# ZhengyiLuo/PULSE

Hardware: NVIDIA H100
Metric: env-steps/sec at 16384 humanoid envs, 1/2/4/8 H100; obs-kernel HBM GB/s (higher is better)
Workload: dtype bf16 GEMM operands, fp32 accumulate / master weights / observations

## Files before the change

pulse_b200/csrc/gemm_kernel.inc:

```
#if PULSE_GEMM_GROUPED
#define PULSE_GEMM_FIRST(member) grp.p[0].member
#define PULSE_GEMM_W wl
#define PULSE_GEMM_SELECT(w)                                                                                         \
  int pi = 0;                                                                                                        \
  while (pi + 1 < grp.count && (w) >= grp.p[pi].item_end) ++pi;                                                      \
  const GemmProblem& P = grp.p[pi];                                                                                  \
  const int wl = (w) - (pi == 0 ? 0 : grp.p[pi - 1].item_end);                                                       \
  const CUtensorMap& map_a = P.map_a;                                                                                \
  const CUtensorMap& map_b = P.map_b;                                                                                \
  const CUtensorMap& map_c = P.map_c;                                                                                \
  const CUtensorMap& map_p = P.map_p;                                                                                \
  const int tma_out = P.tma_out;                                                                                     \
  const pulse_gemm_epilogue_t& ep = P.ep;                                                                            \
  const int M = P.M, N = P.N, K = P.K, kb_per_split = P.kb_per_split;                                                \
  const int tiles_n = (N + BN - 1) / BN, tiles_m = (M + BM - 1) / BM;                                                \
  const int tiles = tiles_m * tiles_n;                                                                               \
  const int num_kb_total = (K + BK - 1) / BK;                                                                        \
  (void)map_a; (void)map_b; (void)map_c; (void)map_p; (void)tma_out; (void)ep; (void)M; (void)N; (void)tiles_n; (void)kb_per_split; (void)num_kb_total;
#else
#define PULSE_GEMM_FIRST(member) member
#define PULSE_GEMM_W w
#define PULSE_GEMM_SELECT(w)
#endif

#if PULSE_GEMM_GROUPED
template <bool A_MN, bool B_MN, int MODE>
__global__ void __launch_bounds__(kThreads, 1) gemm_bf16_grouped_kernel(const __grid_constant__ GemmGroup grp) {
#else
template <bool A_MN, bool B_MN, int MODE>
__global__ void __launch_bounds__(kThreads, 1) gemm_bf16_kernel(const __grid_constant__ CUtensorMap map_a,
                                                                const __grid_constant__ CUtensorMap map_b,
                                                                const __grid_constant__ CUtensorMap map_c,
                                                                const __grid_constant__ CUtensorMap map_p,
                                                                const pulse_gemm_epilogue_t ep, int M, int N, int K,
                                                                int kb_per_split, int splits, int tma_out) {
#endif
  constexpr bool kFwd = MODE == kModeGeneric || MODE == kModeFwd;
  constexpr bool kDgrad = MODE == kModeGeneric || MODE == kModeDgrad || MODE == kModeDgradVec;
  constexpr bool kGateVec = MODE == kModeGeneric || MODE == kModeDgradVec;
  constexpr bool kAccum = MODE == kModeGeneric || MODE == kModeWgrad;
  constexpr bool kBf16Out = MODE != kModeWgrad;
  constexpr bool kRegEpi = MODE == kModeFwd || MODE == kModeDgrad;
  extern __shared__ unsigned char gsm_raw[];
  GemmSmem& sm = *reinterpret_cast<GemmSmem*>((reinterpret_cast<uintptr_t>(gsm_raw) + 1023) & ~static_cast<uintptr_t>(1023));
  const int warp = threadIdx.x >> 5, lane = threadIdx.x & 31;
  const int work0 = static_cast<int>(blockIdx.x);
  const int work_stride = static_cast<int>(gridDim.x);
#if PULSE_GEMM_GROUPED
  const int total = grp.total_items;
#else
  const int tiles_n = (N + BN - 1) / BN, tiles_m = (M + BM - 1) / BM;
  const int tiles = tiles_m * tiles_n;
  const int total = tiles * splits;
  const int num_kb_total = (K + BK - 1) / BK;
#endif
  if (threadIdx.x == 0) PULSE_TRACE(0);

  if (threadIdx.x == 0) {
#pragma unroll
    for (int s = 0; s < kStages; ++s) {
      g_mbar_init(&sm.full[s], 1);
      g_mbar_init(&sm.empty[s], kConsumerWarps);
    }
    asm volatile("fence.mbarrier_init.release.cluster;\n" ::: "memory");
    asm volatile("prefetch.tensormap [%0];\n" ::"l"(&PULSE_GEMM_FIRST(map_a)) : "memory");
    asm volatile("prefetch.tensormap [%0];\n" ::"l"(&PULSE_GEMM_FIRST(map_b)) : "memory");
  }
  __syncthreads();
  if (threadIdx.x == 0) PULSE_TRACE(1);
  asm volatile("griddepcontrol.launch_dependents;\n" ::: "memory");

  if (warp < 4) {
    if (warp == 0 && lane == 0) {
      asm volatile("griddepcontrol.wait;\n" ::: "memory");
      PULSE_TRACE(2);
      int it = 0;
      for (int w = work0; w < total; w += work_stride) {
        PULSE_GEMM_SELECT(w)
        const int split = PULSE_GEMM_W / tiles, t = PULSE_GEMM_W - split * tiles;
        const int m0 = (t / tiles_n) * BM, n0 = (t % tiles_n) * BN;
        const int kb0 = split * kb_per_split;
        const int num_kb = min(kb_per_split, num_kb_total - kb0);
        for (int kb = 0; kb < num_kb; ++kb, ++it) {
          const int s = it % kStages;
          g_mbar_wait(&sm.empty[s], ((it / kStages) & 1) ^ 1);
          g_mbar_expect_tx(&sm.full[s], kStageBytesA + kStageBytesB);
          const int kk = (kb0 + kb) * BK;
          if (A_MN) {
            tma_load_2d(sm.a[s], &map_a, m0, kk, &sm.full[s]);
            tma_load_2d(sm.a[s] + 8192, &map_a, m0 + 64, kk, &sm.full[s]);
          } else {
            tma_load_2d(sm.a[s], &map_a, kk, m0, &sm.full[s]);
          }
          if (B_MN) {
            tma_load_2d(sm.b[s], &map_b, n0, kk, &sm.full[s]);
            tma_load_2d(sm.b[s] + 8192, &map_b, n0 + 64, kk, &sm.full[s]);
          } else {
            tma_load_2d(sm.b[s], &map_b, kk, n0, &sm.full[s]);
          }
        }
      }
    }
  } else {
    const int wg = (warp >> 2) - 1;
    const int ew = warp - 4;
    const int quarter = wg * 2 + (warp & 1);
    const int chalf = (warp >> 1) & 1;
    float* red_stage = sm.red[ew];
    float* acc_s = sm.acc[wg];
    asm volatile("griddepcontrol.wait;\n" ::: "memory");
    int it = 0, lw = 0;
    for (int w = work0; w < total; w += work_stride, ++lw) {
      PULSE_GEMM_SELECT(w)
      const int split = PULSE_GEMM_W / tiles, t = PULSE_GEMM_W - split * tiles;
      const int m0 = (t / tiles_n) * BM, n0 = (t % tiles_n) * BN;
      const int kb0 = split * kb_per_split;
      const int num_kb = min(kb_per_split, num_kb_total - kb0);
      const bool reg_epi = kRegEpi && tma_out;
      const int r0 = (warp & 3) * 16 + (lane >> 2);
      const int row = m0 + quarter * 32 + lane;
      const bool row_ok = row < M;
      const bool gate_fast = (MODE == kModeGeneric || MODE == kModeDgrad) && ep.gate != nullptr && ep.gate_mask == nullptr && ep.gate_mode == PULSE_ACT_RELU && (ep.ldg & 7) == 0 && n0 + chalf * kCols + kCols <= N;
      unsigned gmask[8] = {};
      const bool gate_bits = kDgrad && ep.gate_mask != nullptr;
      if (gate_bits && reg_epi) {
#pragma unroll
        for (int c = 0; c < 4; ++c) {
#pragma unroll
          for (int h = 0; h < 2; ++h) {
            const int r = m0 + wg * 64 + r0 + 8 * h;
            if (r < M && n0 + c * 32 < N) gmask[2 * c + h] = __ldg(ep.gate_mask + static_cast<long long>((n0 >> 5) + c) * ep.ld_gmask + r);
          }
        }
      } else if (gate_bits && row_ok) {
#pragma unroll
        for (int cc = 0; cc < kChunks; ++cc) {
          const int col = n0 + (chalf * kChunks + cc) * 32;
          if (col < N) gmask[cc] = __ldg(ep.gate_mask + static_cast<long long>(col >> 5) * ep.ld_gmask + row);
        }
      }
      if (gate_fast && row_ok) {
        const uint4* g = reinterpret_cast<const uint4*>(reinterpret_cast<const __nv_bfloat16*>(ep.gate) + static_cast<long long>(row) * ep.ldg +
                                                        n0 + chalf * kCols);
        uint4 u[kChunks * 4];
#pragma unroll
        for (int i = 0; i < kChunks * 4; ++i) u[i] = __ldg(g + i);
#pragma unroll
        for (int i = 0; i < kChunks * 4; ++i) {
          const unsigned wds[4] = {u[i].x, u[i].y, u[i].z, u[i].w};
#pragma unroll
          for (int q = 0; q < 4; ++q) {
            const unsigned pos = (((wds[q] & 0x7fff7fffu) + 0x7fff7fffu) & ~wds[q]) & 0x80008000u;
            gmask[i >> 2] |= (pos >> 15) << ((i & 3) * 4 + q);
          }
        }
      }
      const bool gate_vec = kGateVec && ep.gate != nullptr && !gate_fast && !gate_bits && (ep.ldg & 7) == 0;
      uint4 gq[4] = {};
      auto gate_fetch = [&](int cc) {
        const int c0 = n0 + cc * 32;
        if (gate_vec && row_ok && c0 + 32 <= N) {
          const uint4* g = reinterpret_cast<const uint4*>(reinterpret_cast<const __nv_bfloat16*>(ep.gate) + static_cast<long long>(row) * ep.ldg + c0);
#pragma unroll
          for (int q = 0; q < 4; ++q) gq[q] = __ldg(g + q);
        }
      };
      gate_fetch(chalf * kChunks);
      float bias_l[kChunks] = {};
      if (reg_epi && kFwd && ep.bias != nullptr) {
        const int t = (warp & 3) * 32 + lane;
        sm.bias[wg][t] = n0 + t < N ? __ldg(ep.bias + n0 + t) : 0.0f;
      } else if (kFwd && ep.bias != nullptr) {
#pragma unroll
        for (int cc = 0; cc < kChunks; ++cc) {
          const int col = n0 + (chalf * kChunks + cc) * 32 + lane;
          if (col < N) bias_l[cc] = __ldg(ep.bias + col);
        }
      }

      float d[64];
#pragma unroll
      for (int i = 0; i < 64; ++i) d[i] = 0.0f;
      acc_fence(d);
      int prev_s = -1;
      for (int kb = 0; kb < num_kb; ++kb, ++it) {
        const int s = it % kStages;
        g_mbar_wait(&sm.full[s], (it / kStages) & 1);
        if (it == 0 && ew == 0 && lane == 0) PULSE_TRACE(3);
        wgmma_fence();
        const unsigned a_addr = s_u32(sm.a[s]) + static_cast<unsigned>(wg) * 8192u, b_addr = s_u32(sm.b[s]);
#pragma unroll
        for (int k = 0; k < BK / MMA_K; ++k) {
          const unsigned long long da = A_MN ? gmma_desc(a_addr + k * 2048, 8192) : gmma_desc(a_addr + k * 32, 16);
          const unsigned long long db = B_MN ? gmma_desc(b_addr + k * 2048, 8192) : gmma_desc(b_addr + k * 32, 16);
          wgmma_m64n128<A_MN ? 1 : 0, B_MN ? 1 : 0>(d, da, db, (kb | k) != 0 ? 1u : 0u);
        }
        wgmma_commit();
        wgmma_wait<1>();
        if (prev_s >= 0 && lane == 0) g_mbar_arrive(&sm.empty[prev_s]);
        prev_s = s;
      }
      wgmma_wait<0>();
      acc_fence(d);
      if (lane == 0) g_mbar_arrive(&sm.empty[prev_s]);
      if (ew == 0 && lane == 0 && lw < 3) PULSE_TRACE(4 + lw);

      if (kRegEpi && (warp & 3) == 0 && lane == 0) asm volatile("cp.async.bulk.wait_group.read 0;\n" ::: "memory");
      wg_sync(wg);
      float sq = 0.0f;

      if (reg_epi) {
        const int q = lane & 3;
        if (ep.alpha != 1.0f) {
#pragma unroll
          for (int i = 0; i < 64; ++i) d[i] *= ep.alpha;
        }
        if (kFwd && ep.bias != nullptr) {
          const float* bs = sm.bias[wg] + 2 * q;
#pragma unroll
          for (int j = 0; j < BN / 8; ++j) {
            const float2 b = *reinterpret_cast<const float2*>(bs + 8 * j);
            d[4 * j] += b.x; d[4 * j + 1] += b.y; d[4 * j + 2] += b.x; d[4 * j + 3] += b.y;
          }
        }
        if (kFwd && ep.relu_mask != nullptr) {
          unsigned wd[4][2];
#pragma unroll
          for (int c = 0; c < 4; ++c) {
#pragma unroll
            for (int h = 0; h < 2; ++h) {
              unsigned b = 0u;
#pragma unroll
              for (int jj = 0; jj < 4; ++jj)
#pragma unroll
                for (int e = 0; e < 2; ++e) b |= (d[4 * (4 * c + jj) + 2 * h + e] > 0.0f ? 1u : 0u) << (8 * jj + e);
              wd[c][h] = b << (2 * q);
            }
          }
          const bool up2 = (q & 2) != 0, up1 = (q & 1) != 0;
          unsigned wf[2];
#pragma unroll
          for (int h = 0; h < 2; ++h) {
            unsigned w2[2];
#pragma unroll
            for (int k = 0; k < 2; ++k) w2[k] = (up2 ? wd[k + 2][h] : wd[k][h]) | __shfl_xor_sync(0xffffffffu, up2 ? wd[k][h] : wd[k + 2][h], 2);
            wf[h] = (up1 ? w2[1] : w2[0]) | __shfl_xor_sync(0xffffffffu, up1 ? w2[0] : w2[1], 1);
          }
          const int col0 = n0 + 32 * q;
          if (col0 < N) {
            const unsigned valid = N - col0 >= 32 ? 0xffffffffu : (1u << (N - col0)) - 1u;
#pragma unroll
            for (int h = 0; h < 2; ++h) {
              const int r = m0 + wg * 64 + r0 + 8 * h;
              if (r < M) ep.relu_mask[static_cast<long long>(col0 >> 5) * ep.ld_rmask + r] = wf[h] & valid;
            }
          }
        }
        if (gate_bits) {
#pragma unroll
          for (int c = 0; c < 4; ++c) {
#pragma unroll
            for (int h = 0; h < 2; ++h) {
              const unsigned mk = gmask[2 * c + h] >> (2 * q);
#pragma unroll
              for (int jj = 0; jj < 4; ++jj)
#pragma unroll
                for (int e = 0; e < 2; ++e) {
                  float& x = d[4 * (4 * c + jj) + 2 * h + e];
                  x = ((mk >> (8 * jj + e)) & 1u) ? x : 0.0f;
                }
            }
          }
        }
        if (kDgrad && ep.sumsq != nullptr) {
#pragma unroll
          for (int i = 0; i < 64; ++i) sq = fmaf(d[i], d[i], sq);
        }
        const unsigned stage = s_u32(acc_s);
        const bool pre = kFwd && ep.preact != nullptr;
        if (!kFwd || ep.act == PULSE_ACT_NONE) stage_tile_bf16<PULSE_ACT_NONE>(d, stage, pre, n0, N);
        else if (ep.act == PULSE_ACT_RELU) stage_tile_bf16<PULSE_ACT_RELU>(d, stage, pre, n0, N);
        else stage_tile_bf16<PULSE_ACT_SILU>(d, stage, pre, n0, N);
        asm volatile("fence.proxy.async.shared::cta;\n" ::: "memory");
        wg_sync(wg);
        if (ew == 0 && lane == 0 && lw < 3) PULSE_TRACE(16 + 2 * lw);
        if ((warp & 3) == 0 && lane == 0 && m0 + wg * 64 < M) {
#pragma unroll
          for (int b = 0; b < 2; ++b) {
            if (n0 + 64 * b >= N) continue;
            tma_store_2d(&map_c, stage + b * 8192, n0 + 64 * b, m0 + wg * 64);
            if (pre) tma_store_2d(&map_p, stage + 16384 + b * 8192, n0 + 64 * b, m0 + wg * 64);
          }
          asm volatile("cp.async.bulk.commit_group;\n" ::: "memory");
        }
        if (kDgrad && ep.sumsq != nullptr) add_sumsq(ep.sumsq, sq);
        if (ew == 0 && lane == 0 && lw < 3) PULSE_TRACE(17 + 2 * lw);
        continue;
      }

      {
#pragma unroll
        for (int j = 0; j < BN / 8; ++j) {
          const int col = 8 * j + 2 * (lane & 3);
#pragma unroll
          for (int h = 0; h < 2; ++h) {
            const int r = r0 + 8 * h;
            const int rb = r & 31;
            float* blk = acc_s + ((r >> 5) * 4 + (col >> 5)) * 1024;
            const int unit = ((col & 31) >> 2) ^ (rb & 7);
            *reinterpret_cast<float2*>(blk + rb * 32 + unit * 4 + (col & 3)) = make_float2(d[4 * j + 2 * h], d[4 * j + 2 * h + 1]);
          }
        }
      }
      if (MODE == kModeWgrad && tma_out) asm volatile("fence.proxy.async.shared::cta;\n" ::: "memory");
      wg_sync(wg);
      if (ew == 0 && lane == 0 && lw < 3) PULSE_TRACE(16 + 2 * lw);

      float* outf = ep.out_f32 != nullptr ? ep.out_f32 + static_cast<long long>(ep.accumulate ? 0 : split) * ep.split_stride : nullptr;
#pragma unroll 1
      for (int c = chalf * kChunks; c < chalf * kChunks + kChunks; ++c) {
        const int col0 = n0 + c * 32;
        const bool full = col0 + 32 <= N;
        float* blk = acc_s + ((quarter & 1) * 4 + c) * 1024;
        if (MODE == kModeWgrad && tma_out) {
          if (lane == 0) {
            asm volatile("cp.reduce.async.bulk.tensor.2d.global.shared::cta.add.tile.bulk_group [%0, {%2, %3}], [%1];\n" ::"l"(&map_c),
                         "r"(s_u32(blk)), "r"(col0), "r"(m0 + quarter * 32)
                         : "memory");
            asm volatile("cp.async.bulk.commit_group;\n" ::: "memory");
          }
          continue;
        }
        float v[32];
        {
          const float4* b4 = reinterpret_cast<const float4*>(blk) + lane * 8;
#pragma unroll
          for (int u = 0; u < 8; ++u) {
            const float4 x = b4[u ^ (lane & 7)];
            v[4 * u] = x.x; v[4 * u + 1] = x.y; v[4 * u + 2] = x.z; v[4 * u + 3] = x.w;
          }
        }
        if (MODE != kModeWgrad && ep.alpha != 1.0f) {
#pragma unroll
          for (int i = 0; i < 32; ++i) v[i] *= ep.alpha;
        }
        if (kFwd && ep.bias != nullptr) {
          float bl = bias_l[0];
#pragma unroll
          for (int cc = 1; cc < kChunks; ++cc) bl = (c % kChunks) == cc ? bias_l[cc] : bl;
#pragma unroll
          for (int i = 0; i < 32; ++i) v[i] += __shfl_sync(0xffffffffu, bl, i);
        }
        if (kFwd && ep.preact != nullptr) {
          if (full && (ep.ldp & 7) == 0) {
            store_block_bf16(reinterpret_cast<uint4*>(red_stage), v,
                             reinterpret_cast<__nv_bfloat16*>(ep.preact) + static_cast<long long>(m0 + quarter * 32) * ep.ldp + col0, ep.ldp,
                             M - (m0 + quarter * 32), lane);
          } else if (row_ok) {
            __nv_bfloat16* p = reinterpret_cast<__nv_bfloat16*>(ep.preact) + static_cast<long long>(row) * ep.ldp + col0;
#pragma unroll
            for (int i = 0; i < 32; ++i)
              if (col0 + i < N) p[i] = __float2bfloat16(v[i]);
          }
        }
        if (kFwd && ep.relu_mask != nullptr && row_ok) {
          unsigned word = 0u;
#pragma unroll
          for (int i = 0; i < 32; ++i) word |= ((col0 + i < N && v[i] > 0.0f) ? 1u : 0u) << i;
          if (col0 < N) ep.relu_mask[static_cast<long long>(col0 >> 5) * ep.ld_rmask + row] = word;
        }
        if (kFwd && ep.act != PULSE_ACT_NONE) {
#pragma unroll
          for (int i = 0; i < 32; ++i) v[i] = act_apply(v[i], ep.act);
        }
        if (gate_bits) {
          unsigned mk = gmask[0];
#pragma unroll
          for (int cc = 1; cc < kChunks; ++cc) mk = (c % kChunks) == cc ? gmask[cc] : mk;
#pragma unroll
          for (int i = 0; i < 32; ++i) v[i] = ((mk >> i) & 1u) ? v[i] : 0.0f;
        } else if (gate_fast) {
          unsigned mk = gmask[0];
#pragma unroll
          for (int cc = 1; cc < kChunks; ++cc) mk = (c % kChunks) == cc ? gmask[cc] : mk;
#pragma unroll
          for (int i = 0; i < 32; ++i) v[i] = ((mk >> ((i >> 1) + 16 * (i & 1))) & 1u) ? v[i] : 0.0f;
        } else if (kDgrad && ep.gate != nullptr && row_ok) {
          const __nv_bfloat16* g = reinterpret_cast<const __nv_bfloat16*>(ep.gate) + static_cast<long long>(row) * ep.ldg + col0;
          if (full && (gate_vec || (ep.ldg & 7) == 0)) {
#pragma unroll
            for (int i = 0; i < 32; i += 8) {
              const uint4 u = gate_vec ? gq[i >> 3] : __ldg(reinterpret_cast<const uint4*>(g + i));
              const __nv_bfloat162* h = reinterpret_cast<const __nv_bfloat162*>(&u);
#pragma unroll
              for (int q = 0; q < 4; ++q) {
                const float2 f = __bfloat1622float2(h[q]);
                v[i + 2 * q] *= act_grad(f.x, ep.gate_mode);
                v[i + 2 * q + 1] *= act_grad(f.y, ep.gate_mode);
              }
            }
          } else {
#pragma unroll
            for (int i = 0; i < 32; ++i)
              if (col0 + i < N) v[i] *= act_grad(__bfloat162float(g[i]), ep.gate_mode);
          }
        }
        if (gate_vec && c != chalf * kChunks + kChunks - 1) gate_fetch(c + 1);
        if (kDgrad && ep.sumsq != nullptr && row_ok) {
#pragma unroll
          for (int i = 0; i < 32; ++i)
            if (full || col0 + i < N) sq = fmaf(v[i], v[i], sq);
        }
        if (kDgrad && ep.colsum != nullptr) {
          float wv[32];
#pragma unroll
          for (int i = 0; i < 32; ++i) wv[i] = row_ok ? v[i] : 0.0f;
#pragma unroll
          for (int half = 16; half >= 1; half >>= 1) {
            const bool upper = (lane & half) != 0;
#pragma unroll
            for (int i = 0; i < half; ++i) {
              const float mine = upper ? wv[i + half] : wv[i];
              const float send = upper ? wv[i] : wv[i + half];
              wv[i] = mine + __shfl_xor_sync(0xffffffffu, send, half);
            }
          }
          if (col0 + lane < N) atomicAdd(ep.colsum + col0 + lane, wv[0]);
        }
        if (kAccum && outf != nullptr && ep.accumulate) {
#pragma unroll
          for (int hr = 0; hr < 2; ++hr) {
            if ((lane >> 4) == hr) {
#pragma unroll
              for (int i = 0; i < 32; ++i) red_stage[(lane & 15) * 33 + i] = v[i];
            }
            __syncwarp();
            const int rbase = m0 + quarter * 32 + hr * 16;
            const int rows_here = min(16, M - rbase);
            if (col0 + lane < N) {
              float* p = outf + static_cast<long long>(rbase) * ep.ldf + col0 + lane;
              for (int rr = 0; rr < rows_here; ++rr) atomicAdd(p + static_cast<long long>(rr) * ep.ldf, red_stage[rr * 33 + lane]);
            }
            __syncwarp();
          }
        } else if (outf != nullptr && row_ok) {
          float* p = outf + static_cast<long long>(row) * ep.ldf + col0;
          if (full && (ep.ldf & 3) == 0 && (reinterpret_cast<uintptr_t>(outf) & 15u) == 0) {
#pragma unroll
            for (int i = 0; i < 32; i += 4) *reinterpret_cast<float4*>(p + i) = make_float4(v[i], v[i + 1], v[i + 2], v[i + 3]);
          } else {
#pragma unroll
            for (int i = 0; i < 32; ++i)
              if (col0 + i < N) p[i] = v[i];
          }
        }
        if (kBf16Out && ep.out != nullptr) {
          if (full && (ep.ldo & 7) == 0) {
            store_block_bf16(reinterpret_cast<uint4*>(red_stage), v,
                             reinterpret_cast<__nv_bfloat16*>(ep.out) + static_cast<long long>(m0 + quarter * 32) * ep.ldo + col0, ep.ldo,
                             M - (m0 + quarter * 32), lane);
          } else if (row_ok) {
            __nv_bfloat16* p = reinterpret_cast<__nv_bfloat16*>(ep.out) + static_cast<long long>(row) * ep.ldo + col0;
#pragma unroll
            for (int i = 0; i < 32; ++i)
              if (col0 + i < N) p[i] = __float2bfloat16(v[i]);
          }
        }
        if (kFwd && ep.out_t != nullptr && row_ok) {
#pragma unroll
          for (int i = 0; i < 32; ++i)
            if (col0 + i < N)
              reinterpret_cast<__nv_bfloat16*>(ep.out_t)[static_cast<long long>(col0 + i) * ep.ldot + row] = __float2bfloat16(v[i]);
        }
      }
      if (MODE == kModeWgrad && tma_out) {
        if (lane == 0) asm volatile("cp.async.bulk.wait_group.read 0;\n" ::: "memory");
        __syncwarp();
      }
      if (kDgrad && ep.sumsq != nullptr) add_sumsq(ep.sumsq, sq);
      if (ew == 0 && lane == 0 && lw < 3) PULSE_TRACE(17 + 2 * lw);
    }
  }
  if ((MODE == kModeWgrad || kRegEpi) && warp >= 4 && lane == 0) asm volatile("cp.async.bulk.wait_group 0;\n" ::: "memory");
  if (threadIdx.x == 0) PULSE_TRACE(10);
}


#undef PULSE_GEMM_FIRST
#undef PULSE_GEMM_W
#undef PULSE_GEMM_SELECT
```

pulse_b200/csrc/gemm_wgmma.cu:

```cuda
#include <cuda.h>
#include <stdlib.h>
#include <string.h>
#include <cuda_bf16.h>

#include "pulse_common.cuh"

namespace pulse {
namespace {

#ifndef PULSE_GEMM_VARIANT
#define PULSE_GEMM_VARIANT 0
#endif
constexpr int BM = 128, BN = 128, BK = 64, MMA_K = 16;
constexpr int kConsumerWarps = 8;
constexpr int kThreads = 128 + 32 * kConsumerWarps;
constexpr int kCols = 64;
constexpr int kChunks = kCols / 32;
constexpr int kStages = 4;
constexpr unsigned kStageBytesA = BM * BK * 2;
constexpr unsigned kStageBytesB = BN * BK * 2;

struct __align__(1024) GemmSmem {
  unsigned char a[kStages][kStageBytesA];
  unsigned char b[kStages][kStageBytesB];
  float acc[2][64 * BN];
  float red[kConsumerWarps][16 * 33];
  float bias[2][BN];
  unsigned long long full[kStages];
  unsigned long long empty[kStages];
};

__device__ __forceinline__ unsigned s_u32(const void* p) { return static_cast<unsigned>(__cvta_generic_to_shared(p)); }
__device__ __forceinline__ void g_mbar_init(unsigned long long* bar, unsigned count) {
  asm volatile("mbarrier.init.shared::cta.b64 [%0], %1;\n" ::"r"(s_u32(bar)), "r"(count));
}
__device__ __forceinline__ void g_mbar_expect_tx(unsigned long long* bar, unsigned bytes) {
  asm volatile("mbarrier.arrive.expect_tx.shared::cta.b64 _, [%0], %1;\n" ::"r"(s_u32(bar)), "r"(bytes) : "memory");
}
__device__ __forceinline__ void g_mbar_arrive(unsigned long long* bar) {
  asm volatile("mbarrier.arrive.shared::cta.b64 _, [%0];\n" ::"r"(s_u32(bar)) : "memory");
}
__device__ __forceinline__ bool g_mbar_try(unsigned long long* bar, unsigned parity) {
  unsigned ok;
  asm volatile(
      "{\n\t.reg .pred p;\n\t"
      "mbarrier.try_wait.parity.shared::cta.b64 p, [%1], %2;\n\t"
      "selp.u32 %0, 1, 0, p;\n\t}\n"
      : "=r"(ok)
      : "r"(s_u32(bar)), "r"(parity)
      : "memory");
  return ok != 0;
}
__device__ __forceinline__ void g_mbar_wait(unsigned long long* bar, unsigned parity) {
  for (int spin = 0; spin < (1 << 26); ++spin)
    if (g_mbar_try(bar, parity)) return;
  __trap();
}
__device__ __forceinline__ void tma_load_2d(void* smem_dst, const CUtensorMap* map, int c0, int c1, unsigned long long* bar) {
  asm volatile("cp.async.bulk.tensor.2d.shared::cluster.global.mbarrier::complete_tx::bytes [%0], [%1, {%3, %4}], [%2];\n" ::"r"(
                   s_u32(smem_dst)),
               "l"(map), "r"(s_u32(bar)), "r"(c0), "r"(c1)
               : "memory");
}
__device__ __forceinline__ void tma_store_2d(const CUtensorMap* map, unsigned smem_src, int c0, int c1) {
  asm volatile("cp.async.bulk.tensor.2d.global.shared::cta.bulk_group [%0, {%2, %3}], [%1];\n" ::"l"(map), "r"(smem_src), "r"(c0), "r"(c1)
               : "memory");
}
__device__ __forceinline__ void stmatrix_x4(unsigned addr, const unsigned (&r)[4]) {
  asm volatile("stmatrix.sync.aligned.m8n8.x4.shared.b16 [%0], {%1, %2, %3, %4};\n" ::"r"(addr), "r"(r[0]), "r"(r[1]), "r"(r[2]), "r"(r[3])
               : "memory");
}
__device__ __forceinline__ unsigned bf16x2_bits(__nv_bfloat162 h) { return *reinterpret_cast<unsigned*>(&h); }
__device__ __forceinline__ void add_sumsq(double* sumsq, float sq) {
#pragma unroll
  for (int o = 16; o > 0; o >>= 1) sq += __shfl_xor_sync(0xffffffffu, sq, o);
  if ((threadIdx.x & 31) == 0) atomicAdd(sumsq, static_cast<double>(sq));
}
__device__ __forceinline__ void wg_sync(int wg) { asm volatile("bar.sync %0, 128;\n" ::"r"(1 + wg) : "memory"); }

__device__ __forceinline__ unsigned long long gmma_desc(unsigned smem_addr, unsigned lbo) {
  unsigned long long d = 0;
  d |= static_cast<unsigned long long>((smem_addr >> 4) & 0x3fffu);
  d |= static_cast<unsigned long long>((lbo >> 4) & 0x3fffu) << 16;
  d |= static_cast<unsigned long long>(1024u >> 4) << 32;
  d |= static_cast<unsigned long long>(1u) << 62;
  return d;
}
__device__ __forceinline__ void wgmma_fence() { asm volatile("wgmma.fence.sync.aligned;\n" ::: "memory"); }
__device__ __forceinline__ void wgmma_commit() { asm volatile("wgmma.commit_group.sync.aligned;\n" ::: "memory"); }
template <int N>
__device__ __forceinline__ void wgmma_wait() { asm volatile("wgmma.wait_group.sync.aligned %0;\n" ::"n"(N) : "memory"); }
__device__ __forceinline__ void acc_fence(float (&d)[64]) {
#pragma unroll
  for (int i = 0; i < 64; ++i) asm volatile("" : "+f"(d[i])::"memory");
}
template <int TA, int TB>
__device__ __forceinline__ void wgmma_m64n128(float (&d)[64], unsigned long long da, unsigned long long db, unsigned accumulate) {
  asm volatile(
      "{\n\t.reg .pred p;\n\t"
      "setp.ne.b32 p, %66, 0;\n\t"
      "wgmma.mma_async.sync.aligned.m64n128k16.f32.bf16.bf16 "
      "{%0, %1, %2, %3, %4, %5, %6, %7, %8, %9, %10, %11, %12, %13, %14, %15, %16, %17, %18, %19, %20, %21, %22, %23, %24, %25, %26, "
      "%27, %28, %29, %30, %31, %32, %33, %34, %35, %36, %37, %38, %39, %40, %41, %42, %43, %44, %45, %46, %47, %48, %49, %50, %51, "
      "%52, %53, %54, %55, %56, %57, %58, %59, %60, %61, %62, %63}, "
      "%64, %65, p, 1, 1, %67, %68;\n\t}\n"
      : "+f"(d[0]), "+f"(d[1]), "+f"(d[2]), "+f"(d[3]), "+f"(d[4]), "+f"(d[5]), "+f"(d[6]), "+f"(d[7]),
        "+f"(d[8]), "+f"(d[9]), "+f"(d[10]), "+f"(d[11]), "+f"(d[12]), "+f"(d[13]), "+f"(d[14]), "+f"(d[15]),
        "+f"(d[16]), "+f"(d[17]), "+f"(d[18]), "+f"(d[19]), "+f"(d[20]), "+f"(d[21]), "+f"(d[22]), "+f"(d[23]),
        "+f"(d[24]), "+f"(d[25]), "+f"(d[26]), "+f"(d[27]), "+f"(d[28]), "+f"(d[29]), "+f"(d[30]), "+f"(d[31]),
        "+f"(d[32]), "+f"(d[33]), "+f"(d[34]), "+f"(d[35]), "+f"(d[36]), "+f"(d[37]), "+f"(d[38]), "+f"(d[39]),
        "+f"(d[40]), "+f"(d[41]), "+f"(d[42]), "+f"(d[43]), "+f"(d[44]), "+f"(d[45]), "+f"(d[46]), "+f"(d[47]),
        "+f"(d[48]), "+f"(d[49]), "+f"(d[50]), "+f"(d[51]), "+f"(d[52]), "+f"(d[53]), "+f"(d[54]), "+f"(d[55]),
        "+f"(d[56]), "+f"(d[57]), "+f"(d[58]), "+f"(d[59]), "+f"(d[60]), "+f"(d[61]), "+f"(d[62]), "+f"(d[63])
      : "l"(da), "l"(db), "r"(accumulate), "n"(TA), "n"(TB)
      : "memory");
}

__device__ __forceinline__ float act_apply(float x, int act) {
  if (act == PULSE_ACT_RELU) return fmaxf(x, 0.0f);
  if (act == PULSE_ACT_SILU) return __fdividef(x, 1.0f + __expf(-x));
  return x;
}
__device__ __forceinline__ float act_grad(float g, int mode) {
  if (mode == PULSE_ACT_RELU) return g > 0.0f ? 1.0f : 0.0f;
  if (mode == PULSE_ACT_SILU) {
    const float s = __fdividef(1.0f, 1.0f + __expf(-g));
    return s * (1.0f + g * (1.0f - s));
  }
  return 1.0f;
}


__device__ __forceinline__ void store_block_bf16(uint4* st, const float (&v)[32], __nv_bfloat16* base, long long ld, int rows_valid, int lane) {
  const int sw = (lane >> 1) & 3;
#pragma unroll
  for (int q = 0; q < 4; ++q) {
    const int i = 8 * q;
    __nv_bfloat162 h0 = __floats2bfloat162_rn(v[i], v[i + 1]), h1 = __floats2bfloat162_rn(v[i + 2], v[i + 3]);
    __nv_bfloat162 h2 = __floats2bfloat162_rn(v[i + 4], v[i + 5]), h3 = __floats2bfloat162_rn(v[i + 6], v[i + 7]);
    uint4 u;
    u.x = *reinterpret_cast<unsigned*>(&h0);
    u.y = *reinterpret_cast<unsigned*>(&h1);
    u.z = *reinterpret_cast<unsigned*>(&h2);
    u.w = *reinterpret_cast<unsigned*>(&h3);
    st[lane * 4 + (q ^ sw)] = u;
  }
  __syncwarp();
  __nv_bfloat16* obase = base + (lane & 3) * 8;
#pragma unroll
  for (int it = 0; it < 4; ++it) {
    const int rr = it * 8 + (lane >> 2);
    const uint4 val = st[rr * 4 + ((lane & 3) ^ ((rr >> 1) & 3))];
    if (rr < rows_valid) *reinterpret_cast<uint4*>(obase + static_cast<long long>(rr) * ld) = val;
  }
  __syncwarp();
}

#if PULSE_GEMM_VARIANT == 3
__device__ long long g_gemm_trace[32];
#define PULSE_TRACE(slot)                                          \
  do {                                                             \
    if (blockIdx.x == 0) g_gemm_trace[slot] = clock64();           \
  } while (0)
#else
#define PULSE_TRACE(slot) \
  do {                    \
  } while (0)
#endif

__device__ __forceinline__ __nv_bfloat162 silu_bf16x2(__nv_bfloat162 z) {
  float2 f = __bfloat1622float2(z);
  f.x = __fdividef(f.x, 1.0f + __expf(-f.x));
  f.y = __fdividef(f.y, 1.0f + __expf(-f.y));
  return __floats2bfloat162_rn(f.x, f.y);
}

template <int ACT>
__device__ __forceinline__ void stage_tile_bf16(const float (&d)[64], unsigned stage, bool pre, int n0, int N) {
  const int lane = threadIdx.x & 31, warp = threadIdx.x >> 5;
  const unsigned srow = stage + ((warp & 3) * 16 + ((lane >> 3) & 1) * 8 + (lane & 7)) * 128;
  const int sj = lane >> 4;
  const __nv_bfloat162 zero2 = __float2bfloat162_rn(0.0f);
#pragma unroll
  for (int j = 0; j < BN / 8; j += 2) {
    const bool full_half = n0 + 64 * (j >> 3) + 64 <= N;
    unsigned o[4], p[4];
#pragma unroll
    for (int k = 0; k < 4; ++k) {
      const int i = 4 * (j + (k >> 1)) + 2 * (k & 1);
      __nv_bfloat162 h = __floats2bfloat162_rn(d[i], d[i + 1]);
      p[k] = bf16x2_bits(h);
      if (ACT == PULSE_ACT_RELU) h = __hmax2(h, zero2);
      if (ACT == PULSE_ACT_SILU) h = full_half ? silu_bf16x2(h) : __floats2bfloat162_rn(act_apply(d[i], ACT), act_apply(d[i + 1], ACT));
      o[k] = bf16x2_bits(h);
    }
    const unsigned addr = srow + (j >> 3) * 8192 + ((((j & 7) + sj) ^ (lane & 7)) << 4);
    stmatrix_x4(addr, o);
    if (pre) stmatrix_x4(addr + 16384, p);
  }
}

enum : int { kModeGeneric = 0, kModeFwd = 1, kModeDgrad = 2, kModeWgrad = 3, kModeDgradVec = 4 };

constexpr int kMaxGroup = 4;
struct GemmProblem {
  CUtensorMap map_a, map_b, map_c, map_p;
  pulse_gemm_epilogue_t ep;
  int M, N, K, kb_per_split;
  int item_end;
  int tma_out;
  int pad[2];
};
struct GemmGroup {
  GemmProblem p[kMaxGroup];
  int count, total_items;
};

#define PULSE_GEMM_GROUPED 0
#include "gemm_kernel.inc"
#undef PULSE_GEMM_GROUPED
#define PULSE_GEMM_GROUPED 1
#include "gemm_kernel.inc"
#undef PULSE_GEMM_GROUPED

typedef CUresult (*EncodeTiledFn)(CUtensorMap*, CUtensorMapDataType, cuuint32_t, void*, const cuuint64_t*, const cuuint64_t*,
                                  const cuuint32_t*, const cuuint32_t*, CUtensorMapInterleave, CUtensorMapSwizzle,
                                  CUtensorMapL2promotion, CUtensorMapFloatOOBfill);
EncodeTiledFn get_encode_fn() {
  static EncodeTiledFn fn = nullptr;
  if (fn == nullptr) {
    void* p = nullptr;
    cudaDriverEntryPointQueryResult q;
    if (cudaGetDriverEntryPoint("cuTensorMapEncodeTiled", &p, cudaEnableDefault, &q) == cudaSuccess && q == cudaDriverEntryPointSuccess)
      fn = reinterpret_cast<EncodeTiledFn>(p);
  }
  return fn;
}

bool make_map(CUtensorMap* map, const void* base, long long rows, long long cols, long long ld, unsigned box_rows) {
  EncodeTiledFn fn = get_encode_fn();
  if (fn == nullptr) return false;
  cuuint64_t dims[2] = {static_cast<cuuint64_t>(cols), static_cast<cuuint64_t>(rows)};
  cuuint64_t strides[1] = {static_cast<cuuint64_t>(ld) * 2};
  cuuint32_t box[2] = {BK, box_rows};
  cuuint32_t estr[2] = {1, 1};
  return fn(map, CU_TENSOR_MAP_DATA_TYPE_BFLOAT16, 2, const_cast<void*>(base), dims, strides, box, estr, CU_TENSOR_MAP_INTERLEAVE_NONE,
            CU_TENSOR_MAP_SWIZZLE_128B, CU_TENSOR_MAP_L2_PROMOTION_L2_256B, CU_TENSOR_MAP_FLOAT_OOB_FILL_NONE) == CUDA_SUCCESS;
}

bool make_map_c(CUtensorMap* map, const float* base, long long rows, long long cols, long long ld) {
  EncodeTiledFn fn = get_encode_fn();
  if (fn == nullptr) return false;
  cuuint64_t dims[2] = {static_cast<cuuint64_t>(cols), static_cast<cuuint64_t>(rows)};
  cuuint64_t strides[1] = {static_cast<cuuint64_t>(ld) * 4};
  cuuint32_t box[2] = {32, 32};
  cuuint32_t estr[2] = {1, 1};
  return fn(map, CU_TENSOR_MAP_DATA_TYPE_FLOAT32, 2, const_cast<float*>(base), dims, strides, box, estr, CU_TENSOR_MAP_INTERLEAVE_NONE,
            CU_TENSOR_MAP_SWIZZLE_128B, CU_TENSOR_MAP_L2_PROMOTION_NONE, CU_TENSOR_MAP_FLOAT_OOB_FILL_NONE) == CUDA_SUCCESS;
}
bool tma_reduce_ok(const pulse_gemm_epilogue_t& ep) {
  return ep.out_f32 != nullptr && ep.accumulate && (ep.ldf % 4) == 0 && (reinterpret_cast<uintptr_t>(ep.out_f32) % 16) == 0;
}
bool tma_rows_ok(const void* base, long long ld) { return (ld % 8) == 0 && (reinterpret_cast<uintptr_t>(base) % 16) == 0; }

int epilogue_maps(int mode, const pulse_gemm_epilogue_t& ep, long long m, long long n, CUtensorMap* map_c, CUtensorMap* map_p, int* tma_out) {
  memset(map_c, 0, sizeof(*map_c));
  memset(map_p, 0, sizeof(*map_p));
  *tma_out = 0;
  if (mode == kModeWgrad) {
    if (!tma_reduce_ok(ep)) return PULSE_OK;
    if (!make_map_c(map_c, ep.out_f32, m, n, ep.ldf)) {
      set_error("pulse_gemm_bf16: cuTensorMapEncodeTiled failed for the fp32 output");
      return PULSE_ERR_CUDA;
    }
    *tma_out = 1;
    return PULSE_OK;
  }
  if ((mode != kModeFwd && mode != kModeDgrad) || (n % 8) != 0 || ep.out == nullptr || ep.out_f32 != nullptr || ep.out_t != nullptr || ep.gate != nullptr ||
      ep.colsum != nullptr || !tma_rows_ok(ep.out, ep.ldo) || (ep.preact != nullptr && !tma_rows_ok(ep.preact, ep.ldp)))
    return PULSE_OK;
  if (!make_map(map_c, ep.out, m, n, ep.ldo, 64) || (ep.preact != nullptr && !make_map(map_p, ep.preact, m, n, ep.ldp, 64))) {
    set_error("pulse_gemm_bf16: cuTensorMapEncodeTiled failed for the bf16 output");
    return PULSE_ERR_CUDA;
  }
  *tma_out = 1;
  return PULSE_OK;
}

constexpr size_t kSmemBytes = sizeof(GemmSmem) + 1024;

int gemm_num_sms(bool honour_limit) {
  static int num_sms = 0, limited = 0;
  if (num_sms == 0) {
    int dev = 0;
    if (cudaGetDevice(&dev) != cudaSuccess || cudaDeviceGetAttribute(&num_sms, cudaDevAttrMultiProcessorCount, dev) != cudaSuccess) return 0;
    limited = num_sms;
    const char* e = getenv("PULSE_GEMM_SMS");
    if (e != nullptr && atoi(e) >= 1 && atoi(e) < num_sms) limited = atoi(e);
  }
  return honour_limit ? limited : num_sms;
}

template <bool A_MN, bool B_MN, int MODE>
int launch_gemm(const CUtensorMap& map_a, const CUtensorMap& map_b, const pulse_gemm_epilogue_t& ep, int m, int n, int k, int splits,
                int kb_per_split, cudaStream_t stream) {
  static bool attr_set = false;
  CUtensorMap map_c, map_p;
  int tma_out = 0;
  const int rc = epilogue_maps(MODE, ep, m, n, &map_c, &map_p, &tma_out);
  if (rc != PULSE_OK) return rc;
  if (!attr_set) {
    PULSE_CUDA_OK(cudaFuncSetAttribute(gemm_bf16_kernel<A_MN, B_MN, MODE>, cudaFuncAttributeMaxDynamicSharedMemorySize, (int)kSmemBytes));
    attr_set = true;
  }
  const int num_sms = gemm_num_sms(true);
  PULSE_REQUIRE(num_sms > 0, "pulse_gemm_bf16: cannot query the device's SM count");
  const long long total = static_cast<long long>((n + BN - 1) / BN) * ((m + BM - 1) / BM) * splits;
  const unsigned grid = static_cast<unsigned>(total < num_sms ? total : num_sms);
  static int use_pdl = -1;
  if (use_pdl < 0) {
    const char* e = getenv("PULSE_GEMM_PDL");
    use_pdl = (e != nullptr && e[0] == '0') ? 0 : 1;
  }
  cudaLaunchConfig_t cfg = {};
  cfg.gridDim = dim3(grid, 1, 1);
  cfg.blockDim = dim3(kThreads, 1, 1);
  cfg.dynamicSmemBytes = kSmemBytes;
  cfg.stream = stream;
  cudaLaunchAttribute attr[1];
  int na = 0;
  if (use_pdl) {
    attr[na].id = cudaLaunchAttributeProgrammaticStreamSerialization;
    attr[na].val.programmaticStreamSerializationAllowed = 1;
    ++na;
  }
  cfg.attrs = attr;
  cfg.numAttrs = na;
  PULSE_CUDA_OK(cudaLaunchKernelEx(&cfg, gemm_bf16_kernel<A_MN, B_MN, MODE>, map_a, map_b, map_c, map_p, ep, m, n, k, kb_per_split, splits, tma_out));
  PULSE_LAUNCH_OK("gemm_bf16_kernel");
  return PULSE_OK;
}

template <bool A_MN, bool B_MN, int MODE>
int launch_gemm_grouped(const GemmGroup& grp, cudaStream_t stream) {
  static bool attr_set = false;
  if (!attr_set) {
    PULSE_CUDA_OK(cudaFuncSetAttribute(gemm_bf16_grouped_kernel<A_MN, B_MN, MODE>, cudaFuncAttributeMaxDynamicSharedMemorySize, (int)kSmemBytes));
    attr_set = true;
  }
  const int num_sms = gemm_num_sms(false);
  PULSE_REQUIRE(num_sms > 0, "pulse_gemm_bf16_grouped: cannot query the device's SM count");
  const unsigned grid = static_cast<unsigned>(grp.total_items < num_sms ? grp.total_items : num_sms);
  cudaLaunchConfig_t cfg = {};
  cfg.gridDim = dim3(grid, 1, 1);
  cfg.blockDim = dim3(kThreads, 1, 1);
  cfg.dynamicSmemBytes = kSmemBytes;
  cfg.stream = stream;
  cudaLaunchAttribute attr[1];
  attr[0].id = cudaLaunchAttributeProgrammaticStreamSerialization;
  attr[0].val.programmaticStreamSerializationAllowed = 1;
  cfg.attrs = attr;
  cfg.numAttrs = 1;
  PULSE_CUDA_OK(cudaLaunchKernelEx(&cfg, gemm_bf16_grouped_kernel<A_MN, B_MN, MODE>, grp));
  PULSE_LAUNCH_OK("gemm_bf16_grouped_kernel");
  return PULSE_OK;
}

int epilogue_mode(const pulse_gemm_epilogue_t* ep) {
  const bool want_fwd = ep->bias || ep->act != PULSE_ACT_NONE || ep->preact || ep->out_t || ep->relu_mask;
  const bool want_dgrad = ep->gate || ep->colsum || ep->sumsq || ep->gate_mask;
  const bool want_accum = ep->accumulate != 0;
  if (!want_dgrad && !want_accum) return kModeFwd;
  if (!want_fwd && !want_accum) return (ep->gate && ep->gate_mode != PULSE_ACT_RELU) ? kModeDgradVec : kModeDgrad;
  if (!want_fwd && !want_dgrad && !ep->out) return kModeWgrad;
  return kModeGeneric;
}

}
}

#if PULSE_GEMM_VARIANT == 3
extern "C" int pulse_debug_gemm_trace(long long* out) {
  return cudaMemcpyFromSymbol(out, pulse::g_gemm_trace, sizeof(long long) * 32) == cudaSuccess ? 0 : -2;
}
#endif

extern "C" int pulse_gemm_num_splits(int64_t k, int32_t split_k) {
  const int num_kb = static_cast<int>((k + 63) / 64);
  int splits = split_k < 1 ? 1 : (split_k > num_kb ? num_kb : split_k);
  const int kb_per_split = (num_kb + splits - 1) / splits;
  return (num_kb + kb_per_split - 1) / kb_per_split;
}

extern "C" int pulse_gemm_bf16(const void* a, int64_t lda, const void* b, int64_t ldb, int64_t m, int64_t n, int64_t k,
                               const pulse_gemm_epilogue_t* ep, int32_t split_k, uint32_t flags, void* stream) {
  using namespace pulse;
  PULSE_REQUIRE(a && b && ep, "pulse_gemm_bf16: null argument");
  PULSE_REQUIRE(m > 0 && n > 0 && k > 0, "pulse_gemm_bf16: empty problem %lld x %lld x %lld", (long long)m, (long long)n, (long long)k);
  PULSE_REQUIRE(m < (1ll << 31) && n < (1ll << 31) && k < (1ll << 31), "pulse_gemm_bf16: dimension too large");
  PULSE_REQUIRE((flags & ~3u) == 0, "pulse_gemm_bf16: bad flags");
  const bool a_mn = flags & PULSE_GEMM_A_MN, b_mn = flags & PULSE_GEMM_B_MN;
  PULSE_REQUIRE(lda >= (a_mn ? m : k) && ldb >= (b_mn ? n : k) && (lda % 8) == 0 && (ldb % 8) == 0,
                "pulse_gemm_bf16: leading dimensions must cover the contiguous extent and be multiples of 8 (16-byte rows), got %lld %lld",
                (long long)lda, (long long)ldb);
  PULSE_REQUIRE(aligned16(a) && aligned16(b), "pulse_gemm_bf16: operands must be 16-byte aligned");
  PULSE_REQUIRE(ep->out || ep->out_t || ep->out_f32, "pulse_gemm_bf16: no output requested");
  PULSE_REQUIRE(split_k >= 1, "pulse_gemm_bf16: split_k must be >= 1");
  PULSE_REQUIRE(split_k == 1 || (ep->out_f32 && !ep->out && !ep->out_t && !ep->bias && ep->act == PULSE_ACT_NONE && !ep->gate && !ep->preact && !ep->colsum),
                "pulse_gemm_bf16: split-K only supports plain fp32 outputs (slabs or atomic accumulation)");
  PULSE_REQUIRE(ep->gate == nullptr || ep->gate_mode == PULSE_ACT_RELU || ep->gate_mode == PULSE_ACT_SILU, "pulse_gemm_bf16: bad gate_mode");
  PULSE_REQUIRE((ep->relu_mask == nullptr || ep->ld_rmask >= m) && (ep->gate_mask == nullptr || ep->ld_gmask >= m),
                "pulse_gemm_bf16: mask word rows must hold at least M entries");
  PULSE_REQUIRE(!(ep->gate_mask && ep->gate), "pulse_gemm_bf16: give the ReLU gate either as bf16 activations or as bit words, not both");
  CUtensorMap map_a, map_b;
  const bool ok_a = a_mn ? make_map(&map_a, a, k, m, lda, 64) : make_map(&map_a, a, m, k, lda, BM);
  const bool ok_b = b_mn ? make_map(&map_b, b, k, n, ldb, 64) : make_map(&map_b, b, n, k, ldb, BN);
  if (!ok_a || !ok_b) {
    set_error("pulse_gemm_bf16: cuTensorMapEncodeTiled failed (driver entry point missing or bad strides)");
    return PULSE_ERR_CUDA;
  }
  const int num_kb = static_cast<int>((k + BK - 1) / BK);
  const int splits = pulse_gemm_num_splits(k, split_k);
  const int kb_per_split = (num_kb + splits - 1) / splits;
  cudaStream_t st = static_cast<cudaStream_t>(stream);
  const int mode = epilogue_mode(ep);
  const int mi = (int)m, ni = (int)n, ki = (int)k;
#define PULSE_GEMM_DISPATCH(AM, BM_)                                                                                        \
  switch (mode) {                                                                                                           \
    case kModeFwd: return launch_gemm<AM, BM_, kModeFwd>(map_a, map_b, *ep, mi, ni, ki, splits, kb_per_split, st);             \
    case kModeDgrad: return launch_gemm<AM, BM_, kModeDgrad>(map_a, map_b, *ep, mi, ni, ki, splits, kb_per_split, st);         \
    case kModeWgrad: return launch_gemm<AM, BM_, kModeWgrad>(map_a, map_b, *ep, mi, ni, ki, splits, kb_per_split, st);         \
    case kModeDgradVec: return launch_gemm<AM, BM_, kModeDgradVec>(map_a, map_b, *ep, mi, ni, ki, splits, kb_per_split, st);   \
    default: return launch_gemm<AM, BM_, kModeGeneric>(map_a, map_b, *ep, mi, ni, ki, splits, kb_per_split, st);               \
  }
  if (a_mn && b_mn) { PULSE_GEMM_DISPATCH(true, true) }
  if (a_mn) { PULSE_GEMM_DISPATCH(true, false) }
  if (b_mn) { PULSE_GEMM_DISPATCH(false, true) }
  PULSE_GEMM_DISPATCH(false, false)
#undef PULSE_GEMM_DISPATCH
}

extern "C" int pulse_gemm_bf16_nt(const void* a, int64_t lda, const void* b, int64_t ldb, int64_t m, int64_t n, int64_t k,
                                  const pulse_gemm_epilogue_t* ep, int32_t split_k, void* stream) {
  return pulse_gemm_bf16(a, lda, b, ldb, m, n, k, ep, split_k, 0u, stream);
}

extern "C" int pulse_gemm_bf16_grouped(const pulse_gemm_problem_t* problems, int32_t count, uint32_t flags, void* stream) {
  using namespace pulse;
  PULSE_REQUIRE(problems != nullptr && count >= 1 && count <= kMaxGroup, "pulse_gemm_bf16_grouped: 1..%d problems", kMaxGroup);
  PULSE_REQUIRE((flags & ~3u) == 0, "pulse_gemm_bf16_grouped: bad flags");
  const bool a_mn = flags & PULSE_GEMM_A_MN, b_mn = flags & PULSE_GEMM_B_MN;
  int mode = -1;
  for (int i = 0; i < count; ++i) {
    const pulse_gemm_problem_t& q = problems[i];
    PULSE_REQUIRE(q.a && q.b, "pulse_gemm_bf16_grouped: null operand in problem %d", i);
    PULSE_REQUIRE(q.m > 0 && q.n > 0 && q.k > 0 && q.m < (1ll << 31) && q.n < (1ll << 31) && q.k < (1ll << 31), "pulse_gemm_bf16_grouped: bad shape in problem %d", i);
    PULSE_REQUIRE(q.lda >= (a_mn ? q.m : q.k) && q.ldb >= (b_mn ? q.n : q.k) && (q.lda % 8) == 0 && (q.ldb % 8) == 0,
                  "pulse_gemm_bf16_grouped: leading dimensions of problem %d must cover the contiguous extent and be multiples of 8", i);
    PULSE_REQUIRE(aligned16(q.a) && aligned16(q.b), "pulse_gemm_bf16_grouped: operands of problem %d must be 16-byte aligned", i);
    PULSE_REQUIRE(q.ep.out || q.ep.out_t || q.ep.out_f32, "pulse_gemm_bf16_grouped: problem %d has no output", i);
    PULSE_REQUIRE(q.split_k >= 1, "pulse_gemm_bf16_grouped: split_k must be >= 1");
    PULSE_REQUIRE(q.split_k == 1 || (q.ep.out_f32 && q.ep.accumulate && !q.ep.out && !q.ep.out_t && !q.ep.bias && q.ep.act == PULSE_ACT_NONE && !q.ep.gate &&
                                     !q.ep.preact && !q.ep.colsum),
                  "pulse_gemm_bf16_grouped: split-K only with fp32 atomic accumulation");
    const int mq = epilogue_mode(&q.ep);
    PULSE_REQUIRE(mode < 0 || mq == mode, "pulse_gemm_bf16_grouped: problem %d needs a different epilogue specialisation than problem 0", i);
    mode = mq;
  }
  PULSE_REQUIRE(mode == kModeFwd || mode == kModeDgrad || mode == kModeWgrad, "pulse_gemm_bf16_grouped: forward, ReLU-dgrad and wgrad groups only");
  PULSE_REQUIRE((mode == kModeFwd && !a_mn && !b_mn) || (mode == kModeDgrad && !a_mn && b_mn) || (mode == kModeWgrad && a_mn && b_mn),
                "pulse_gemm_bf16_grouped: operand majors do not match the group kind (fwd K/K, dgrad K/MN, wgrad MN/MN)");
  GemmGroup grp;
  memset(&grp, 0, sizeof(grp));
  grp.count = count;
  long long items = 0;
  for (int i = 0; i < count; ++i) {
    const pulse_gemm_problem_t& q = problems[i];
    GemmProblem& g = grp.p[i];
    const bool ok_a = a_mn ? make_map(&g.map_a, q.a, q.k, q.m, q.lda, 64) : make_map(&g.map_a, q.a, q.m, q.k, q.lda, BM);
    const bool ok_b = b_mn ? make_map(&g.map_b, q.b, q.k, q.n, q.ldb, 64) : make_map(&g.map_b, q.b, q.n, q.k, q.ldb, BN);
    if (!ok_a || !ok_b) {
      set_error("pulse_gemm_bf16_grouped: cuTensorMapEncodeTiled failed for problem %d", i);
      return PULSE_ERR_CUDA;
    }
    g.ep = q.ep;
    const int rc = epilogue_maps(mode, q.ep, q.m, q.n, &g.map_c, &g.map_p, &g.tma_out);
    if (rc != PULSE_OK) return rc;
    g.M = static_cast<int>(q.m);
    g.N = static_cast<int>(q.n);
    g.K = static_cast<int>(q.k);
    const int num_kb = static_cast<int>((q.k + BK - 1) / BK);
    const int splits = pulse_gemm_num_splits(q.k, q.split_k);
    g.kb_per_split = (num_kb + splits - 1) / splits;
    items += static_cast<long long>((q.n + BN - 1) / BN) * ((q.m + BM - 1) / BM) * splits;
    PULSE_REQUIRE(items < (1ll << 30), "pulse_gemm_bf16_grouped: too many work items");
    g.item_end = static_cast<int>(items);
  }
  grp.total_items = static_cast<int>(items);
  cudaStream_t st = static_cast<cudaStream_t>(stream);
  if (mode == kModeFwd) return launch_gemm_grouped<false, false, kModeFwd>(grp, st);
  if (mode == kModeDgrad) return launch_gemm_grouped<false, true, kModeDgrad>(grp, st);
  return launch_gemm_grouped<true, true, kModeWgrad>(grp, st);
}
```

Baseline: 1.892 million.

## Deepen GEMM TMA ring for register-epilogue modes and add TMA fp32 output path

Templates the GEMM kernels on the pipeline stage count and selects a 5- or 6-stage smem ring for forward and ReLU-dgrad GEMMs that use the register-resident TMA-store epilogue. It drops the staged smem accumulator buffers in those instantiations to make room for the deeper ring. It also adds a TMA bulk-store path for plain fp32 forward outputs, including split slabs. Instrumentation records barrier wait clocks. The aim is to hide more load latency and cut epilogue store cost, at the price of more template instantiations, higher smem per block and an env-var override.

```diff
diff --git a/pulse_b200/csrc/gemm_kernel.inc b/pulse_b200/csrc/gemm_kernel.inc
--- a/pulse_b200/csrc/gemm_kernel.inc
+++ b/pulse_b200/csrc/gemm_kernel.inc
@@ -24,10 +24,10 @@
 #endif
 
 #if PULSE_GEMM_GROUPED
-template <bool A_MN, bool B_MN, int MODE>
+template <bool A_MN, bool B_MN, int MODE, int S>
 __global__ void __launch_bounds__(kThreads, 1) gemm_bf16_grouped_kernel(const __grid_constant__ GemmGroup grp) {
 #else
-template <bool A_MN, bool B_MN, int MODE>
+template <bool A_MN, bool B_MN, int MODE, int S>
 __global__ void __launch_bounds__(kThreads, 1) gemm_bf16_kernel(const __grid_constant__ CUtensorMap map_a,
                                                                 const __grid_constant__ CUtensorMap map_b,
                                                                 const __grid_constant__ CUtensorMap map_c,
@@ -41,8 +41,11 @@
   constexpr bool kAccum = MODE == kModeGeneric || MODE == kModeWgrad;
   constexpr bool kBf16Out = MODE != kModeWgrad;
   constexpr bool kRegEpi = MODE == kModeFwd || MODE == kModeDgrad;
+  constexpr bool kStaged = S == kStages;
+  static_assert(kStaged || kRegEpi, "deep-ring instantiations run the register-resident epilogue only");
+  constexpr bool kPreRoom = sizeof(GemmSmem<S>::epi[0]) >= 32768;
   extern __shared__ unsigned char gsm_raw[];
-  GemmSmem& sm = *reinterpret_cast<GemmSmem*>((reinterpret_cast<uintptr_t>(gsm_raw) + 1023) & ~static_cast<uintptr_t>(1023));
+  GemmSmem<S>& sm = *reinterpret_cast<GemmSmem<S>*>((reinterpret_cast<uintptr_t>(gsm_raw) + 1023) & ~static_cast<uintptr_t>(1023));
   const int warp = threadIdx.x >> 5, lane = threadIdx.x & 31;
   const int work0 = static_cast<int>(blockIdx.x);
   const int work_stride = static_cast<int>(gridDim.x);
@@ -54,11 +57,11 @@
   const int total = tiles * splits;
   const int num_kb_total = (K + BK - 1) / BK;
 #endif
-  if (threadIdx.x == 0) PULSE_TRACE(0);
+  if (threadIdx.x == 0) PULSE_TRACE_START();
 
   if (threadIdx.x == 0) {
 #pragma unroll
-    for (int s = 0; s < kStages; ++s) {
+    for (int s = 0; s < S; ++s) {
       g_mbar_init(&sm.full[s], 1);
       g_mbar_init(&sm.empty[s], kConsumerWarps);
     }
@@ -74,16 +77,19 @@
     if (warp == 0 && lane == 0) {
       asm volatile("griddepcontrol.wait;\n" ::: "memory");
       PULSE_TRACE(2);
-      int it = 0;
-      for (int w = work0; w < total; w += work_stride) {
+      int it = 0, lw = 0;
+      for (int w = work0; w < total; w += work_stride, ++lw) {
         PULSE_GEMM_SELECT(w)
         const int split = PULSE_GEMM_W / tiles, t = PULSE_GEMM_W - split * tiles;
         const int m0 = (t / tiles_n) * BM, n0 = (t % tiles_n) * BN;
         const int kb0 = split * kb_per_split;
         const int num_kb = min(kb_per_split, num_kb_total - kb0);
+        long long empty_clk = 0;
+        (void)empty_clk;
+        if (lw < 3) PULSE_TRACE_SET(25 + lw, num_kb);
         for (int kb = 0; kb < num_kb; ++kb, ++it) {
-          const int s = it % kStages;
-          g_mbar_wait(&sm.empty[s], ((it / kStages) & 1) ^ 1);
+          const int s = it % S;
+          PULSE_RING_WAIT(&sm.empty[s], ((it / S) & 1) ^ 1, empty_clk);
           g_mbar_expect_tx(&sm.full[s], kStageBytesA + kStageBytesB);
           const int kk = (kb0 + kb) * BK;
           if (A_MN) {
@@ -99,6 +105,7 @@
             tma_load_2d(sm.b[s], &map_b, kk, n0, &sm.full[s]);
           }
         }
+        if (lw < 3) PULSE_TRACE_SET(28 + lw, empty_clk);
       }
     }
   } else {
@@ -106,8 +113,12 @@
     const int ew = warp - 4;
     const int quarter = wg * 2 + (warp & 1);
     const int chalf = (warp >> 1) & 1;
-    float* red_stage = sm.red[ew];
-    float* acc_s = sm.acc[wg];
+    float* red_stage = nullptr;
+    float* acc_s = nullptr;
+    if constexpr (kStaged) {
+      red_stage = sm.red[ew];
+      acc_s = sm.epi[wg];
+    }
     asm volatile("griddepcontrol.wait;\n" ::: "memory");
     int it = 0, lw = 0;
     for (int w = work0; w < total; w += work_stride, ++lw) {
@@ -116,11 +127,11 @@
       const int m0 = (t / tiles_n) * BM, n0 = (t % tiles_n) * BN;
       const int kb0 = split * kb_per_split;
       const int num_kb = min(kb_per_split, num_kb_total - kb0);
-      const bool reg_epi = kRegEpi && tma_out;
+      const bool reg_epi = !kStaged || (kRegEpi && tma_out);
       const int r0 = (warp & 3) * 16 + (lane >> 2);
       const int row = m0 + quarter * 32 + lane;
       const bool row_ok = row < M;
-      const bool gate_fast = (MODE == kModeGeneric || MODE == kModeDgrad) && ep.gate != nullptr && ep.gate_mask == nullptr && ep.gate_mode == PULSE_ACT_RELU && (ep.ldg & 7) == 0 && n0 + chalf * kCols + kCols <= N;
+      const bool gate_fast = kStaged && (MODE == kModeGeneric || MODE == kModeDgrad) && ep.gate != nullptr && ep.gate_mask == nullptr && ep.gate_mode == PULSE_ACT_RELU && (ep.ldg & 7) == 0 && n0 + chalf * kCols + kCols <= N;
       unsigned gmask[8] = {};
       const bool gate_bits = kDgrad && ep.gate_mask != nullptr;
       if (gate_bits && reg_epi) {
@@ -155,7 +166,7 @@
           }
         }
       }
-      const bool gate_vec = kGateVec && ep.gate != nullptr && !gate_fast && !gate_bits && (ep.ldg & 7) == 0;
+      const bool gate_vec = kStaged && kGateVec && ep.gate != nullptr && !gate_fast && !gate_bits && (ep.ldg & 7) == 0;
       uint4 gq[4] = {};
       auto gate_fetch = [&](int cc) {
         const int c0 = n0 + cc * 32;
@@ -183,9 +194,11 @@
       for (int i = 0; i < 64; ++i) d[i] = 0.0f;
       acc_fence(d);
       int prev_s = -1;
+      long long full_clk = 0;
+      (void)full_clk;
       for (int kb = 0; kb < num_kb; ++kb, ++it) {
-        const int s = it % kStages;
-        g_mbar_wait(&sm.full[s], (it / kStages) & 1);
+        const int s = it % S;
+        PULSE_RING_WAIT(&sm.full[s], (it / S) & 1, full_clk);
         if (it == 0 && ew == 0 && lane == 0) PULSE_TRACE(3);
         wgmma_fence();
         const unsigned a_addr = s_u32(sm.a[s]) + static_cast<unsigned>(wg) * 8192u, b_addr = s_u32(sm.b[s]);
@@ -203,7 +216,10 @@
       wgmma_wait<0>();
       acc_fence(d);
       if (lane == 0) g_mbar_arrive(&sm.empty[prev_s]);
-      if (ew == 0 && lane == 0 && lw < 3) PULSE_TRACE(4 + lw);
+      if (ew == 0 && lane == 0 && lw < 3) {
+        PULSE_TRACE(4 + lw);
+        PULSE_TRACE_SET(22 + lw, full_clk);
+      }
 
       if (kRegEpi && (warp & 3) == 0 && lane == 0) asm volatile("cp.async.bulk.wait_group.read 0;\n" ::: "memory");
       wg_sync(wg);
@@ -276,8 +292,42 @@
 #pragma unroll
           for (int i = 0; i < 64; ++i) sq = fmaf(d[i], d[i], sq);
         }
-        const unsigned stage = s_u32(acc_s);
-        const bool pre = kFwd && ep.preact != nullptr;
+        if constexpr (kFwd && !kStaged) {
+          if (tma_out == kTmaOutF32) {
+            const unsigned st = s_u32(sm.epi[wg]);
+#pragma unroll
+            for (int hf = 0; hf < 2; ++hf) {
+              if (hf == 1) {
+                if ((warp & 3) == 0 && lane == 0) asm volatile("cp.async.bulk.wait_group.read 0;\n" ::: "memory");
+                wg_sync(wg);
+              }
+#pragma unroll
+              for (int j = 8 * hf; j < 8 * hf + 8; ++j) {
+                const int lc = 8 * j + 2 * q - 64 * hf;
+#pragma unroll
+                for (int h = 0; h < 2; ++h) {
+                  const int r = r0 + 8 * h;
+                  const unsigned addr = st + ((r >> 5) * 2 + (lc >> 5)) * 4096 + (r & 31) * 128 + ((((lc & 31) >> 2) ^ (r & 7)) << 4) + (lc & 3) * 4;
+                  asm volatile("st.shared.v2.f32 [%0], {%1, %2};\n" ::"r"(addr), "f"(d[4 * j + 2 * h]), "f"(d[4 * j + 2 * h + 1]) : "memory");
+                }
+              }
+              asm volatile("fence.proxy.async.shared::cta;\n" ::: "memory");
+              wg_sync(wg);
+              if ((warp & 3) == 0 && lane == 0 && m0 + wg * 64 < M) {
+#pragma unroll
+                for (int blk = 0; blk < 4; ++blk) {
+                  const int col0 = n0 + 64 * hf + 32 * (blk & 1), rw = m0 + wg * 64 + 32 * (blk >> 1);
+                  if (col0 < N && rw < M) tma_store_3d(&map_c, st + blk * 4096, col0, rw, split);
+                }
+                asm volatile("cp.async.bulk.commit_group;\n" ::: "memory");
+              }
+            }
+            if (ew == 0 && lane == 0 && lw < 3) PULSE_TRACE(17 + 2 * lw);
+            continue;
+          }
+        }
+        const unsigned stage = s_u32(sm.epi[wg]);
+        const bool pre = kFwd && kPreRoom && ep.preact != nullptr;
         if (!kFwd || ep.act == PULSE_ACT_NONE) stage_tile_bf16<PULSE_ACT_NONE>(d, stage, pre, n0, N);
         else if (ep.act == PULSE_ACT_RELU) stage_tile_bf16<PULSE_ACT_RELU>(d, stage, pre, n0, N);
         else stage_tile_bf16<PULSE_ACT_SILU>(d, stage, pre, n0, N);
@@ -298,187 +348,189 @@
         continue;
       }
 
-      {
-#pragma unroll
-        for (int j = 0; j < BN / 8; ++j) {
-          const int col = 8 * j + 2 * (lane & 3);
-#pragma unroll
-          for (int h = 0; h < 2; ++h) {
-            const int r = r0 + 8 * h;
-            const int rb = r & 31;
-            float* blk = acc_s + ((r >> 5) * 4 + (col >> 5)) * 1024;
-            const int unit = ((col & 31) >> 2) ^ (rb & 7);
-            *reinterpret_cast<float2*>(blk + rb * 32 + unit * 4 + (col & 3)) = make_float2(d[4 * j + 2 * h], d[4 * j + 2 * h + 1]);
-          }
-        }
-      }
-      if (MODE == kModeWgrad && tma_out) asm volatile("fence.proxy.async.shared::cta;\n" ::: "memory");
-      wg_sync(wg);
-      if (ew == 0 && lane == 0 && lw < 3) PULSE_TRACE(16 + 2 * lw);
-
-      float* outf = ep.out_f32 != nullptr ? ep.out_f32 + static_cast<long long>(ep.accumulate ? 0 : split) * ep.split_stride : nullptr;
-#pragma unroll 1
-      for (int c = chalf * kChunks; c < chalf * kChunks + kChunks; ++c) {
-        const int col0 = n0 + c * 32;
-        const bool full = col0 + 32 <= N;
-        float* blk = acc_s + ((quarter & 1) * 4 + c) * 1024;
+      if constexpr (kStaged) {
+        {
+  #pragma unroll
+          for (int j = 0; j < BN / 8; ++j) {
+            const int col = 8 * j + 2 * (lane & 3);
+  #pragma unroll
+            for (int h = 0; h < 2; ++h) {
+              const int r = r0 + 8 * h;
+              const int rb = r & 31;
+              float* blk = acc_s + ((r >> 5) * 4 + (col >> 5)) * 1024;
+              const int unit = ((col & 31) >> 2) ^ (rb & 7);
+              *reinterpret_cast<float2*>(blk + rb * 32 + unit * 4 + (col & 3)) = make_float2(d[4 * j + 2 * h], d[4 * j + 2 * h + 1]);
+            }
+          }
+        }
+        if (MODE == kModeWgrad && tma_out) asm volatile("fence.proxy.async.shared::cta;\n" ::: "memory");
+        wg_sync(wg);
+        if (ew == 0 && lane == 0 && lw < 3) PULSE_TRACE(16 + 2 * lw);
+
+        float* outf = ep.out_f32 != nullptr ? ep.out_f32 + static_cast<long long>(ep.accumulate ? 0 : split) * ep.split_stride : nullptr;
+  #pragma unroll 1
+        for (int c = chalf * kChunks; c < chalf * kChunks + kChunks; ++c) {
+          const int col0 = n0 + c * 32;
+          const bool full = col0 + 32 <= N;
+          float* blk = acc_s + ((quarter & 1) * 4 + c) * 1024;
+          if (MODE == kModeWgrad && tma_out) {
+            if (lane == 0) {
+              asm volatile("cp.reduce.async.bulk.tensor.2d.global.shared::cta.add.tile.bulk_group [%0, {%2, %3}], [%1];\n" ::"l"(&map_c),
+                           "r"(s_u32(blk)), "r"(col0), "r"(m0 + quarter * 32)
+                           : "memory");
+              asm volatile("cp.async.bulk.commit_group;\n" ::: "memory");
+            }
+            continue;
+          }
+          float v[32];
+          {
+            const float4* b4 = reinterpret_cast<const float4*>(blk) + lane * 8;
+  #pragma unroll
+            for (int u = 0; u < 8; ++u) {
+              const float4 x = b4[u ^ (lane & 7)];
+              v[4 * u] = x.x; v[4 * u + 1] = x.y; v[4 * u + 2] = x.z; v[4 * u + 3] = x.w;
+            }
+          }
+          if (MODE != kModeWgrad && ep.alpha != 1.0f) {
+  #pragma unroll
+            for (int i = 0; i < 32; ++i) v[i] *= ep.alpha;
+          }
+          if (kFwd && ep.bias != nullptr) {
+            float bl = bias_l[0];
+  #pragma unroll
+            for (int cc = 1; cc < kChunks; ++cc) bl = (c % kChunks) == cc ? bias_l[cc] : bl;
+  #pragma unroll
+            for (int i = 0; i < 32; ++i) v[i] += __shfl_sync(0xffffffffu, bl, i);
+          }
+          if (kFwd && ep.preact != nullptr) {
+            if (full && (ep.ldp & 7) == 0) {
+              store_block_bf16(reinterpret_cast<uint4*>(red_stage), v,
+                               reinterpret_cast<__nv_bfloat16*>(ep.preact) + static_cast<long long>(m0 + quarter * 32) * ep.ldp + col0, ep.ldp,
+                               M - (m0 + quarter * 32), lane);
+            } else if (row_ok) {
+              __nv_bfloat16* p = reinterpret_cast<__nv_bfloat16*>(ep.preact) + static_cast<long long>(row) * ep.ldp + col0;
+  #pragma unroll
+              for (int i = 0; i < 32; ++i)
+                if (col0 + i < N) p[i] = __float2bfloat16(v[i]);
+            }
+          }
+          if (kFwd && ep.relu_mask != nullptr && row_ok) {
+            unsigned word = 0u;
+  #pragma unroll
+            for (int i = 0; i < 32; ++i) word |= ((col0 + i < N && v[i] > 0.0f) ? 1u : 0u) << i;
+            if (col0 < N) ep.relu_mask[static_cast<long long>(col0 >> 5) * ep.ld_rmask + row] = word;
+          }
+          if (kFwd && ep.act != PULSE_ACT_NONE) {
+  #pragma unroll
+            for (int i = 0; i < 32; ++i) v[i] = act_apply(v[i], ep.act);
+          }
+          if (gate_bits) {
+            unsigned mk = gmask[0];
+  #pragma unroll
+            for (int cc = 1; cc < kChunks; ++cc) mk = (c % kChunks) == cc ? gmask[cc] : mk;
+  #pragma unroll
+            for (int i = 0; i < 32; ++i) v[i] = ((mk >> i) & 1u) ? v[i] : 0.0f;
+          } else if (gate_fast) {
+            unsigned mk = gmask[0];
+  #pragma unroll
+            for (int cc = 1; cc < kChunks; ++cc) mk = (c % kChunks) == cc ? gmask[cc] : mk;
+  #pragma unroll
+            for (int i = 0; i < 32; ++i) v[i] = ((mk >> ((i >> 1) + 16 * (i & 1))) & 1u) ? v[i] : 0.0f;
+          } else if (kDgrad && ep.gate != nullptr && row_ok) {
+            const __nv_bfloat16* g = reinterpret_cast<const __nv_bfloat16*>(ep.gate) + static_cast<long long>(row) * ep.ldg + col0;
+            if (full && (gate_vec || (ep.ldg & 7) == 0)) {
+  #pragma unroll
+              for (int i = 0; i < 32; i += 8) {
+                const uint4 u = gate_vec ? gq[i >> 3] : __ldg(reinterpret_cast<const uint4*>(g + i));
+                const __nv_bfloat162* h = reinterpret_cast<const __nv_bfloat162*>(&u);
+  #pragma unroll
+                for (int q = 0; q < 4; ++q) {
+                  const float2 f = __bfloat1622float2(h[q]);
+                  v[i + 2 * q] *= act_grad(f.x, ep.gate_mode);
+                  v[i + 2 * q + 1] *= act_grad(f.y, ep.gate_mode);
+                }
+              }
+            } else {
+  #pragma unroll
+              for (int i = 0; i < 32; ++i)
+                if (col0 + i < N) v[i] *= act_grad(__bfloat162float(g[i]), ep.gate_mode);
+            }
+          }
+          if (gate_vec && c != chalf * kChunks + kChunks - 1) gate_fetch(c + 1);
+          if (kDgrad && ep.sumsq != nullptr && row_ok) {
+  #pragma unroll
+            for (int i = 0; i < 32; ++i)
+              if (full || col0 + i < N) sq = fmaf(v[i], v[i], sq);
+          }
+          if (kDgrad && ep.colsum != nullptr) {
+            float wv[32];
+  #pragma unroll
+            for (int i = 0; i < 32; ++i) wv[i] = row_ok ? v[i] : 0.0f;
+  #pragma unroll
+            for (int half = 16; half >= 1; half >>= 1) {
+              const bool upper = (lane & half) != 0;
+  #pragma unroll
+              for (int i = 0; i < half; ++i) {
+                const float mine = upper ? wv[i + half] : wv[i];
+                const float send = upper ? wv[i] : wv[i + half];
+                wv[i] = mine + __shfl_xor_sync(0xffffffffu, send, half);
+              }
+            }
+            if (col0 + lane < N) atomicAdd(ep.colsum + col0 + lane, wv[0]);
+          }
+          if (kAccum && outf != nullptr && ep.accumulate) {
+  #pragma unroll
+            for (int hr = 0; hr < 2; ++hr) {
+              if ((lane >> 4) == hr) {
+  #pragma unroll
+                for (int i = 0; i < 32; ++i) red_stage[(lane & 15) * 33 + i] = v[i];
+              }
+              __syncwarp();
+              const int rbase = m0 + quarter * 32 + hr * 16;
+              const int rows_here = min(16, M - rbase);
+              if (col0 + lane < N) {
+                float* p = outf + static_cast<long long>(rbase) * ep.ldf + col0 + lane;
+                for (int rr = 0; rr < rows_here; ++rr) atomicAdd(p + static_cast<long long>(rr) * ep.ldf, red_stage[rr * 33 + lane]);
+              }
+              __syncwarp();
+            }
+          } else if (outf != nullptr && row_ok) {
+            float* p = outf + static_cast<long long>(row) * ep.ldf + col0;
+            if (full && (ep.ldf & 3) == 0 && (reinterpret_cast<uintptr_t>(outf) & 15u) == 0) {
+  #pragma unroll
+              for (int i = 0; i < 32; i += 4) *reinterpret_cast<float4*>(p + i) = make_float4(v[i], v[i + 1], v[i + 2], v[i + 3]);
+            } else {
+  #pragma unroll
+              for (int i = 0; i < 32; ++i)
+                if (col0 + i < N) p[i] = v[i];
+            }
+          }
+          if (kBf16Out && ep.out != nullptr) {
+            if (full && (ep.ldo & 7) == 0) {
+              store_block_bf16(reinterpret_cast<uint4*>(red_stage), v,
+                               reinterpret_cast<__nv_bfloat16*>(ep.out) + static_cast<long long>(m0 + quarter * 32) * ep.ldo + col0, ep.ldo,
+                               M - (m0 + quarter * 32), lane);
+            } else if (row_ok) {
+              __nv_bfloat16* p = reinterpret_cast<__nv_bfloat16*>(ep.out) + static_cast<long long>(row) * ep.ldo + col0;
+  #pragma unroll
+              for (int i = 0; i < 32; ++i)
+                if (col0 + i < N) p[i] = __float2bfloat16(v[i]);
+            }
+          }
+          if (kFwd && ep.out_t != nullptr && row_ok) {
+  #pragma unroll
+            for (int i = 0; i < 32; ++i)
+              if (col0 + i < N)
+                reinterpret_cast<__nv_bfloat16*>(ep.out_t)[static_cast<long long>(col0 + i) * ep.ldot + row] = __float2bfloat16(v[i]);
+          }
+        }
         if (MODE == kModeWgrad && tma_out) {
-          if (lane == 0) {
-            asm volatile("cp.reduce.async.bulk.tensor.2d.global.shared::cta.add.tile.bulk_group [%0, {%2, %3}], [%1];\n" ::"l"(&map_c),
-                         "r"(s_u32(blk)), "r"(col0), "r"(m0 + quarter * 32)
-                         : "memory");
-            asm volatile("cp.async.bulk.commit_group;\n" ::: "memory");
-          }
-          continue;
-        }
-        float v[32];
-        {
-          const float4* b4 = reinterpret_cast<const float4*>(blk) + lane * 8;
-#pragma unroll
-          for (int u = 0; u < 8; ++u) {
-            const float4 x = b4[u ^ (lane & 7)];
-            v[4 * u] = x.x; v[4 * u + 1] = x.y; v[4 * u + 2] = x.z; v[4 * u + 3] = x.w;
-          }
-        }
-        if (MODE != kModeWgrad && ep.alpha != 1.0f) {
-#pragma unroll
-          for (int i = 0; i < 32; ++i) v[i] *= ep.alpha;
-        }
-        if (kFwd && ep.bias != nullptr) {
-          float bl = bias_l[0];
-#pragma unroll
-          for (int cc = 1; cc < kChunks; ++cc) bl = (c % kChunks) == cc ? bias_l[cc] : bl;
-#pragma unroll
-          for (int i = 0; i < 32; ++i) v[i] += __shfl_sync(0xffffffffu, bl, i);
-        }
-        if (kFwd && ep.preact != nullptr) {
-          if (full && (ep.ldp & 7) == 0) {
-            store_block_bf16(reinterpret_cast<uint4*>(red_stage), v,
-                             reinterpret_cast<__nv_bfloat16*>(ep.preact) + static_cast<long long>(m0 + quarter * 32) * ep.ldp + col0, ep.ldp,
-                             M - (m0 + quarter * 32), lane);
-          } else if (row_ok) {
-            __nv_bfloat16* p = reinterpret_cast<__nv_bfloat16*>(ep.preact) + static_cast<long long>(row) * ep.ldp + col0;
-#pragma unroll
-            for (int i = 0; i < 32; ++i)
-              if (col0 + i < N) p[i] = __float2bfloat16(v[i]);
-          }
-        }
-        if (kFwd && ep.relu_mask != nullptr && row_ok) {
-          unsigned word = 0u;
-#pragma unroll
-          for (int i = 0; i < 32; ++i) word |= ((col0 + i < N && v[i] > 0.0f) ? 1u : 0u) << i;
-          if (col0 < N) ep.relu_mask[static_cast<long long>(col0 >> 5) * ep.ld_rmask + row] = word;
-        }
-        if (kFwd && ep.act != PULSE_ACT_NONE) {
-#pragma unroll
-          for (int i = 0; i < 32; ++i) v[i] = act_apply(v[i], ep.act);
-        }
-        if (gate_bits) {
-          unsigned mk = gmask[0];
-#pragma unroll
-          for (int cc = 1; cc < kChunks; ++cc) mk = (c % kChunks) == cc ? gmask[cc] : mk;
-#pragma unroll
-          for (int i = 0; i < 32; ++i) v[i] = ((mk >> i) & 1u) ? v[i] : 0.0f;
-        } else if (gate_fast) {
-          unsigned mk = gmask[0];
-#pragma unroll
-          for (int cc = 1; cc < kChunks; ++cc) mk = (c % kChunks) == cc ? gmask[cc] : mk;
-#pragma unroll
-          for (int i = 0; i < 32; ++i) v[i] = ((mk >> ((i >> 1) + 16 * (i & 1))) & 1u) ? v[i] : 0.0f;
-        } else if (kDgrad && ep.gate != nullptr && row_ok) {
-          const __nv_bfloat16* g = reinterpret_cast<const __nv_bfloat16*>(ep.gate) + static_cast<long long>(row) * ep.ldg + col0;
-          if (full && (gate_vec || (ep.ldg & 7) == 0)) {
-#pragma unroll
-            for (int i = 0; i < 32; i += 8) {
-              const uint4 u = gate_vec ? gq[i >> 3] : __ldg(reinterpret_cast<const uint4*>(g + i));
-              const __nv_bfloat162* h = reinterpret_cast<const __nv_bfloat162*>(&u);
-#pragma unroll
-              for (int q = 0; q < 4; ++q) {
-                const float2 f = __bfloat1622float2(h[q]);
-                v[i + 2 * q] *= act_grad(f.x, ep.gate_mode);
-                v[i + 2 * q + 1] *= act_grad(f.y, ep.gate_mode);
-              }
-            }
-          } else {
-#pragma unroll
-            for (int i = 0; i < 32; ++i)
-              if (col0 + i < N) v[i] *= act_grad(__bfloat162float(g[i]), ep.gate_mode);
-          }
-        }
-        if (gate_vec && c != chalf * kChunks + kChunks - 1) gate_fetch(c + 1);
-        if (kDgrad && ep.sumsq != nullptr && row_ok) {
-#pragma unroll
-          for (int i = 0; i < 32; ++i)
-            if (full || col0 + i < N) sq = fmaf(v[i], v[i], sq);
-        }
-        if (kDgrad && ep.colsum != nullptr) {
-          float wv[32];
-#pragma unroll
-          for (int i = 0; i < 32; ++i) wv[i] = row_ok ? v[i] : 0.0f;
-#pragma unroll
-          for (int half = 16; half >= 1; half >>= 1) {
-            const bool upper = (lane & half) != 0;
-#pragma unroll
-            for (int i = 0; i < half; ++i) {
-              const float mine = upper ? wv[i + half] : wv[i];
-              const float send = upper ? wv[i] : wv[i + half];
-              wv[i] = mine + __shfl_xor_sync(0xffffffffu, send, half);
-            }
-          }
-          if (col0 + lane < N) atomicAdd(ep.colsum + col0 + lane, wv[0]);
-        }
-        if (kAccum && outf != nullptr && ep.accumulate) {
-#pragma unroll
-          for (int hr = 0; hr < 2; ++hr) {
-            if ((lane >> 4) == hr) {
-#pragma unroll
-              for (int i = 0; i < 32; ++i) red_stage[(lane & 15) * 33 + i] = v[i];
-            }
-            __syncwarp();
-            const int rbase = m0 + quarter * 32 + hr * 16;
-            const int rows_here = min(16, M - rbase);
-            if (col0 + lane < N) {
-              float* p = outf + static_cast<long long>(rbase) * ep.ldf + col0 + lane;
-              for (int rr = 0; rr < rows_here; ++rr) atomicAdd(p + static_cast<long long>(rr) * ep.ldf, red_stage[rr * 33 + lane]);
-            }
-            __syncwarp();
-          }
-        } else if (outf != nullptr && row_ok) {
-          float* p = outf + static_cast<long long>(row) * ep.ldf + col0;
-          if (full && (ep.ldf & 3) == 0 && (reinterpret_cast<uintptr_t>(outf) & 15u) == 0) {
-#pragma unroll
-            for (int i = 0; i < 32; i += 4) *reinterpret_cast<float4*>(p + i) = make_float4(v[i], v[i + 1], v[i + 2], v[i + 3]);
-          } else {
-#pragma unroll
-            for (int i = 0; i < 32; ++i)
-              if (col0 + i < N) p[i] = v[i];
-          }
-        }
-        if (kBf16Out && ep.out != nullptr) {
-          if (full && (ep.ldo & 7) == 0) {
-            store_block_bf16(reinterpret_cast<uint4*>(red_stage), v,
-                             reinterpret_cast<__nv_bfloat16*>(ep.out) + static_cast<long long>(m0 + quarter * 32) * ep.ldo + col0, ep.ldo,
-                             M - (m0 + quarter * 32), lane);
-          } else if (row_ok) {
-            __nv_bfloat16* p = reinterpret_cast<__nv_bfloat16*>(ep.out) + static_cast<long long>(row) * ep.ldo + col0;
-#pragma unroll
-            for (int i = 0; i < 32; ++i)
-              if (col0 + i < N) p[i] = __float2bfloat16(v[i]);
-          }
-        }
-        if (kFwd && ep.out_t != nullptr && row_ok) {
-#pragma unroll
-          for (int i = 0; i < 32; ++i)
-            if (col0 + i < N)
-              reinterpret_cast<__nv_bfloat16*>(ep.out_t)[static_cast<long long>(col0 + i) * ep.ldot + row] = __float2bfloat16(v[i]);
-        }
-      }
-      if (MODE == kModeWgrad && tma_out) {
-        if (lane == 0) asm volatile("cp.async.bulk.wait_group.read 0;\n" ::: "memory");
-        __syncwarp();
-      }
-      if (kDgrad && ep.sumsq != nullptr) add_sumsq(ep.sumsq, sq);
-      if (ew == 0 && lane == 0 && lw < 3) PULSE_TRACE(17 + 2 * lw);
+          if (lane == 0) asm volatile("cp.async.bulk.wait_group.read 0;\n" ::: "memory");
+          __syncwarp();
+        }
+        if (kDgrad && ep.sumsq != nullptr) add_sumsq(ep.sumsq, sq);
+        if (ew == 0 && lane == 0 && lw < 3) PULSE_TRACE(17 + 2 * lw);
+      }
     }
   }
   if ((MODE == kModeWgrad || kRegEpi) && warp >= 4 && lane == 0) asm volatile("cp.async.bulk.wait_group 0;\n" ::: "memory");
diff --git a/pulse_b200/csrc/gemm_wgmma.cu b/pulse_b200/csrc/gemm_wgmma.cu
--- a/pulse_b200/csrc/gemm_wgmma.cu
+++ b/pulse_b200/csrc/gemm_wgmma.cu
@@ -17,18 +17,34 @@
 constexpr int kCols = 64;
 constexpr int kChunks = kCols / 32;
 constexpr int kStages = 4;
+constexpr int kTmaOutF32 = 2;
 constexpr unsigned kStageBytesA = BM * BK * 2;
 constexpr unsigned kStageBytesB = BN * BK * 2;
 
+template <int S>
 struct __align__(1024) GemmSmem {
+  unsigned char a[S][kStageBytesA];
+  unsigned char b[S][kStageBytesB];
+  unsigned char epi[2][S >= 6 ? 16384 : 32768];
+  float bias[2][BN];
+  unsigned long long full[S];
+  unsigned long long empty[S];
+};
+template <>
+struct __align__(1024) GemmSmem<kStages> {
   unsigned char a[kStages][kStageBytesA];
   unsigned char b[kStages][kStageBytesB];
-  float acc[2][64 * BN];
+  float epi[2][64 * BN];
   float red[kConsumerWarps][16 * 33];
   float bias[2][BN];
   unsigned long long full[kStages];
   unsigned long long empty[kStages];
 };
+template <int S>
+constexpr size_t smem_bytes() { return sizeof(GemmSmem<S>) + 1024; }
+constexpr size_t kSmemOptin = 232448;
+static_assert(smem_bytes<kStages>() <= kSmemOptin && smem_bytes<5>() <= kSmemOptin && smem_bytes<6>() <= kSmemOptin,
+              "GEMM shared-memory layout exceeds the per-block opt-in limit");
 
 __device__ __forceinline__ unsigned s_u32(const void* p) { return static_cast<unsigned>(__cvta_generic_to_shared(p)); }
 __device__ __forceinline__ void g_mbar_init(unsigned long long* bar, unsigned count) {
@@ -64,6 +80,11 @@
 }
 __device__ __forceinline__ void tma_store_2d(const CUtensorMap* map, unsigned smem_src, int c0, int c1) {
   asm volatile("cp.async.bulk.tensor.2d.global.shared::cta.bulk_group [%0, {%2, %3}], [%1];\n" ::"l"(map), "r"(smem_src), "r"(c0), "r"(c1)
+               : "memory");
+}
+__device__ __forceinline__ void tma_store_3d(const CUtensorMap* map, unsigned smem_src, int c0, int c1, int c2) {
+  asm volatile("cp.async.bulk.tensor.3d.global.shared::cta.bulk_group [%0, {%2, %3, %4}], [%1];\n" ::"l"(map), "r"(smem_src), "r"(c0), "r"(c1),
+               "r"(c2)
                : "memory");
 }
 __device__ __forceinline__ void stmatrix_x4(unsigned addr, const unsigned (&r)[4]) {
@@ -162,10 +183,34 @@
   do {                                                             \
     if (blockIdx.x == 0) g_gemm_trace[slot] = clock64();           \
   } while (0)
+#define PULSE_TRACE_SET(slot, v)                                   \
+  do {                                                             \
+    if (blockIdx.x == 0) g_gemm_trace[slot] = (v);                 \
+  } while (0)
+#define PULSE_TRACE_START()                                        \
+  do {                                                             \
+    if (blockIdx.x == 0) {                                         \
+      for (int i_ = 1; i_ < 32; ++i_) g_gemm_trace[i_] = 0;        \
+      g_gemm_trace[0] = clock64();                                 \
+    }                                                              \
+  } while (0)
+#define PULSE_RING_WAIT(bar, parity, clk)                          \
+  do {                                                             \
+    const long long t_ = clock64();                                \
+    g_mbar_wait(bar, parity);                                      \
+    clk += clock64() - t_;                                         \
+  } while (0)
 #else
 #define PULSE_TRACE(slot) \
   do {                    \
   } while (0)
+#define PULSE_TRACE_SET(slot, v) \
+  do {                           \
+  } while (0)
+#define PULSE_TRACE_START() \
+  do {                      \
+  } while (0)
+#define PULSE_RING_WAIT(bar, parity, clk) g_mbar_wait(bar, parity)
 #endif
 
 __device__ __forceinline__ __nv_bfloat162 silu_bf16x2(__nv_bfloat162 z) {
@@ -258,12 +303,23 @@
   return fn(map, CU_TENSOR_MAP_DATA_TYPE_FLOAT32, 2, const_cast<float*>(base), dims, strides, box, estr, CU_TENSOR_MAP_INTERLEAVE_NONE,
             CU_TENSOR_MAP_SWIZZLE_128B, CU_TENSOR_MAP_L2_PROMOTION_NONE, CU_TENSOR_MAP_FLOAT_OOB_FILL_NONE) == CUDA_SUCCESS;
 }
+bool make_map_slabs(CUtensorMap* map, const float* base, long long splits, long long rows, long long cols, long long ld, long long split_stride) {
+  EncodeTiledFn fn = get_encode_fn();
+  if (fn == nullptr) return false;
+  cuuint64_t dims[3] = {static_cast<cuuint64_t>(cols), static_cast<cuuint64_t>(rows), static_cast<cuuint64_t>(splits)};
+  cuuint64_t strides[2] = {static_cast<cuuint64_t>(ld) * 4, static_cast<cuuint64_t>(splits > 1 ? split_stride : rows * ld) * 4};
+  cuuint32_t box[3] = {32, 32, 1};
+  cuuint32_t estr[3] = {1, 1, 1};
+  return fn(map, CU_TENSOR_MAP_DATA_TYPE_FLOAT32, 3, const_cast<float*>(base), dims, strides, box, estr, CU_TENSOR_MAP_INTERLEAVE_NONE,
+            CU_TENSOR_MAP_SWIZZLE_128B, CU_TENSOR_MAP_L2_PROMOTION_NONE, CU_TENSOR_MAP_FLOAT_OOB_FILL_NONE) == CUDA_SUCCESS;
+}
 bool tma_reduce_ok(const pulse_gemm_epilogue_t& ep) {
   return ep.out_f32 != nullptr && ep.accumulate && (ep.ldf % 4) == 0 && (reinterpret_cast<uintptr_t>(ep.out_f32) % 16) == 0;
 }
 bool tma_rows_ok(const void* base, long long ld) { return (ld % 8) == 0 && (reinterpret_cast<uintptr_t>(base) % 16) == 0; }
 
-int epilogue_maps(int mode, const pulse_gemm_epilogue_t& ep, long long m, long long n, CUtensorMap* map_c, CUtensorMap* map_p, int* tma_out) {
+int epilogue_maps(int mode, const pulse_gemm_epilogue_t& ep, long long m, long long n, int splits, CUtensorMap* map_c, CUtensorMap* map_p,
+                  int* tma_out) {
   memset(map_c, 0, sizeof(*map_c));
   memset(map_p, 0, sizeof(*map_p));
   *tma_out = 0;
@@ -276,6 +332,16 @@
     *tma_out = 1;
     return PULSE_OK;
   }
+  if (mode == kModeFwd && ep.out_f32 != nullptr && ep.out == nullptr && ep.out_t == nullptr && ep.preact == nullptr && ep.relu_mask == nullptr &&
+      ep.bias == nullptr && ep.act == PULSE_ACT_NONE && ep.alpha == 1.0f && !ep.accumulate && (n % 4) == 0 && (ep.ldf % 4) == 0 &&
+      (reinterpret_cast<uintptr_t>(ep.out_f32) % 16) == 0 && (splits == 1 || (ep.split_stride % 4) == 0)) {
+    if (!make_map_slabs(map_c, ep.out_f32, splits, m, n, ep.ldf, ep.split_stride)) {
+      set_error("pulse_gemm_bf16: cuTensorMapEncodeTiled failed for the fp32 output");
+      return PULSE_ERR_CUDA;
+    }
+    *tma_out = kTmaOutF32;
+    return PULSE_OK;
+  }
   if ((mode != kModeFwd && mode != kModeDgrad) || (n % 8) != 0 || ep.out == nullptr || ep.out_f32 != nullptr || ep.out_t != nullptr || ep.gate != nullptr ||
       ep.colsum != nullptr || !tma_rows_ok(ep.out, ep.ldo) || (ep.preact != nullptr && !tma_rows_ok(ep.preact, ep.ldp)))
     return PULSE_OK;
@@ -286,8 +352,6 @@
   *tma_out = 1;
   return PULSE_OK;
 }
-
-constexpr size_t kSmemBytes = sizeof(GemmSmem) + 1024;
 
 int gemm_num_sms(bool honour_limit) {
   static int num_sms = 0, limited = 0;
@@ -301,18 +365,31 @@
   return honour_limit ? limited : num_sms;
 }
 
-template <bool A_MN, bool B_MN, int MODE>
-int launch_gemm(const CUtensorMap& map_a, const CUtensorMap& map_b, const pulse_gemm_epilogue_t& ep, int m, int n, int k, int splits,
-                int kb_per_split, cudaStream_t stream) {
+int ring_stages(bool reg_epi, bool preact) {
+  const char* e = getenv("PULSE_GEMM_STAGES");
+  const bool force4 = e != nullptr && atoi(e) == kStages;
+  return (!reg_epi || force4) ? kStages : preact ? 5 : 6;
+}
+
+template <typename Kernel>
+int set_smem_once(Kernel kernel, size_t bytes, bool* done) {
+  if (*done) return PULSE_OK;
+  int dev = 0, optin = 0;
+  PULSE_CUDA_OK(cudaGetDevice(&dev));
+  PULSE_CUDA_OK(cudaDeviceGetAttribute(&optin, cudaDevAttrMaxSharedMemoryPerBlockOptin, dev));
+  PULSE_REQUIRE(bytes <= static_cast<size_t>(optin), "pulse_gemm_bf16: the GEMM needs %zu bytes of shared memory per block, the device allows %d",
+                bytes, optin);
+  PULSE_CUDA_OK(cudaFuncSetAttribute(kernel, cudaFuncAttributeMaxDynamicSharedMemorySize, static_cast<int>(bytes)));
+  *done = true;
+  return PULSE_OK;
+}
+
+template <bool A_MN, bool B_MN, int MODE, int S>
+int launch_gemm_ring(const CUtensorMap& map_a, const CUtensorMap& map_b, const CUtensorMap& map_c, const CUtensorMap& map_p,
+                     const pulse_gemm_epilogue_t& ep, int m, int n, int k, int splits, int kb_per_split, int tma_out, cudaStream_t stream) {
   static bool attr_set = false;
-  CUtensorMap map_c, map_p;
-  int tma_out = 0;
-  const int rc = epilogue_maps(MODE, ep, m, n, &map_c, &map_p, &tma_out);
+  const int rc = set_smem_once(gemm_bf16_kernel<A_MN, B_MN, MODE, S>, smem_bytes<S>(), &attr_set);
   if (rc != PULSE_OK) return rc;
-  if (!attr_set) {
-    PULSE_CUDA_OK(cudaFuncSetAttribute(gemm_bf16_kernel<A_MN, B_MN, MODE>, cudaFuncAttributeMaxDynamicSharedMemorySize, (int)kSmemBytes));
-    attr_set = true;
-  }
   const int num_sms = gemm_num_sms(true);
   PULSE_REQUIRE(num_sms > 0, "pulse_gemm_bf16: cannot query the device's SM count");
   const long long total = static_cast<long long>((n + BN - 1) / BN) * ((m + BM - 1) / BM) * splits;
@@ -325,7 +402,7 @@
   cudaLaunchConfig_t cfg = {};
   cfg.gridDim = dim3(grid, 1, 1);
   cfg.blockDim = dim3(kThreads, 1, 1);
-  cfg.dynamicSmemBytes = kSmemBytes;
+  cfg.dynamicSmemBytes = smem_bytes<S>();
   cfg.stream = stream;
   cudaLaunchAttribute attr[1];
   int na = 0;
@@ -336,32 +413,48 @@
   }
   cfg.attrs = attr;
   cfg.numAttrs = na;
-  PULSE_CUDA_OK(cudaLaunchKernelEx(&cfg, gemm_bf16_kernel<A_MN, B_MN, MODE>, map_a, map_b, map_c, map_p, ep, m, n, k, kb_per_split, splits, tma_out));
+  PULSE_CUDA_OK(cudaLaunchKernelEx(&cfg, gemm_bf16_kernel<A_MN, B_MN, MODE, S>, map_a, map_b, map_c, map_p, ep, m, n, k, kb_per_split, splits, tma_out));
   PULSE_LAUNCH_OK("gemm_bf16_kernel");
   return PULSE_OK;
 }
 
 template <bool A_MN, bool B_MN, int MODE>
+int launch_gemm(const CUtensorMap& map_a, const CUtensorMap& map_b, const pulse_gemm_epilogue_t& ep, int m, int n, int k, int splits,
+                int kb_per_split, cudaStream_t stream) {
+  CUtensorMap map_c, map_p;
+  int tma_out = 0;
+  const int rc = epilogue_maps(MODE, ep, m, n, splits, &map_c, &map_p, &tma_out);
+  if (rc != PULSE_OK) return rc;
+  if constexpr (MODE == kModeFwd || MODE == kModeDgrad) {
+    const int s = ring_stages(tma_out != 0, ep.preact != nullptr);
+    if (s == kStages && tma_out == kTmaOutF32) tma_out = 0;
+    if (s == 6) return launch_gemm_ring<A_MN, B_MN, MODE, 6>(map_a, map_b, map_c, map_p, ep, m, n, k, splits, kb_per_split, tma_out, stream);
+    if constexpr (MODE == kModeFwd) {
+      if (s == 5) return launch_gemm_ring<A_MN, B_MN, MODE, 5>(map_a, map_b, map_c, map_p, ep, m, n, k, splits, kb_per_split, tma_out, stream);
+    }
+  }
+  return launch_gemm_ring<A_MN, B_MN, MODE, kStages>(map_a, map_b, map_c, map_p, ep, m, n, k, splits, kb_per_split, tma_out, stream);
+}
+
+template <bool A_MN, bool B_MN, int MODE, int S>
 int launch_gemm_grouped(const GemmGroup& grp, cudaStream_t stream) {
   static bool attr_set = false;
-  if (!attr_set) {
-    PULSE_CUDA_OK(cudaFuncSetAttribute(gemm_bf16_grouped_kernel<A_MN, B_MN, MODE>, cudaFuncAttributeMaxDynamicSharedMemorySize, (int)kSmemBytes));
-    attr_set = true;
-  }
+  const int rc = set_smem_once(gemm_bf16_grouped_kernel<A_MN, B_MN, MODE, S>, smem_bytes<S>(), &attr_set);
+  if (rc != PULSE_OK) return rc;
   const int num_sms = gemm_num_sms(false);
   PULSE_REQUIRE(num_sms > 0, "pulse_gemm_bf16_grouped: cannot query the device's SM count");
   const unsigned grid = static_cast<unsigned>(grp.total_items < num_sms ? grp.total_items : num_sms);
   cudaLaunchConfig_t cfg = {};
   cfg.gridDim = dim3(grid, 1, 1);
   cfg.blockDim = dim3(kThreads, 1, 1);
-  cfg.dynamicSmemBytes = kSmemBytes;
+  cfg.dynamicSmemBytes = smem_bytes<S>();
   cfg.stream = stream;
   cudaLaunchAttribute attr[1];
   attr[0].id = cudaLaunchAttributeProgrammaticStreamSerialization;
   attr[0].val.programmaticStreamSerializationAllowed = 1;
   cfg.attrs = attr;
   cfg.numAttrs = 1;
-  PULSE_CUDA_OK(cudaLaunchKernelEx(&cfg, gemm_bf16_grouped_kernel<A_MN, B_MN, MODE>, grp));
+  PULSE_CUDA_OK(cudaLaunchKernelEx(&cfg, gemm_bf16_grouped_kernel<A_MN, B_MN, MODE, S>, grp));
   PULSE_LAUNCH_OK("gemm_bf16_grouped_kernel");
   return PULSE_OK;
 }
@@ -484,7 +577,7 @@
       return PULSE_ERR_CUDA;
     }
     g.ep = q.ep;
-    const int rc = epilogue_maps(mode, q.ep, q.m, q.n, &g.map_c, &g.map_p, &g.tma_out);
+    const int rc = epilogue_maps(mode, q.ep, q.m, q.n, 1, &g.map_c, &g.map_p, &g.tma_out);
     if (rc != PULSE_OK) return rc;
     g.M = static_cast<int>(q.m);
     g.N = static_cast<int>(q.n);
@@ -498,7 +591,22 @@
   }
   grp.total_items = static_cast<int>(items);
   cudaStream_t st = static_cast<cudaStream_t>(stream);
-  if (mode == kModeFwd) return launch_gemm_grouped<false, false, kModeFwd>(grp, st);
-  if (mode == kModeDgrad) return launch_gemm_grouped<false, true, kModeDgrad>(grp, st);
-  return launch_gemm_grouped<true, true, kModeWgrad>(grp, st);
-}
+  bool reg_epi = true, preact = false;
+  for (int i = 0; i < count; ++i) {
+    reg_epi = reg_epi && grp.p[i].tma_out;
+    preact = preact || problems[i].ep.preact != nullptr;
+  }
+  const int s = ring_stages(mode != kModeWgrad && reg_epi, preact);
+  for (int i = 0; i < count; ++i)
+    if (s == kStages && grp.p[i].tma_out == kTmaOutF32) grp.p[i].tma_out = 0;
+  if (mode == kModeFwd) {
+    if (s == 6) return launch_gemm_grouped<false, false, kModeFwd, 6>(grp, st);
+    if (s == 5) return launch_gemm_grouped<false, false, kModeFwd, 5>(grp, st);
+    return launch_gemm_grouped<false, false, kModeFwd, kStages>(grp, st);
+  }
+  if (mode == kModeDgrad) {
+    if (s == 6) return launch_gemm_grouped<false, true, kModeDgrad, 6>(grp, st);
+    return launch_gemm_grouped<false, true, kModeDgrad, kStages>(grp, st);
+  }
+  return launch_gemm_grouped<true, true, kModeWgrad, kStages>(grp, st);
+}
```

Result: faster. 1.993 million (median of 6 runs) (+5.3%).
